# dusk-network/plonk

Hardware: AMD Instinct MI355X
Metric: prove() wall-clock (ms) at 2^20 gates (lower is better)
Workload: dtype u32 limbs (Fr 256-bit / Fp 384-bit Montgomery)

## Files before the change

### include/plonk_hip.h

```cpp
#ifndef PLONK_HIP_H
#define PLONK_HIP_H
#include <stdint.h>

#ifdef __cplusplus
extern "C" {
#endif

typedef struct plonk_ctx plonk_ctx;

enum {
  PLONK_OK = 0,
  PLONK_ERR_ARG = -1,
  PLONK_ERR_HIP = -2,
  PLONK_ERR_DEGREE = -3,
  PLONK_ERR_NO_SRS = -4,
  PLONK_ERR_NO_GPU = -5,
  PLONK_ERR_UNSAT = -6,
  PLONK_ERR_STATE = -7,
  PLONK_ERR_BYTES = -8,
  PLONK_ERR_DATA = -9,
  PLONK_ERR_POINT = -10,
  PLONK_ERR_NOMEM = -11,
  PLONK_ERR_VERIFY = -12
};

int plonk_ctx_create(plonk_ctx** out, const int* devices, int ndev);
void plonk_ctx_destroy(plonk_ctx* ctx);
const char* plonk_last_error(void);

enum { PLONK_TABLE_AUTO = 0, PLONK_TABLE_WINDOW = 16, PLONK_TABLE_HALFPOS = 128, PLONK_TABLE_BITPOS = 256 };
typedef struct plonk_gpu_config {
  uint32_t struct_size;
  uint32_t reserved;
  uint64_t table_budget_bytes;
  int32_t table_mode;
  int32_t msm_bucket_bits;
  int32_t quotient_domain;
  int32_t wire_commit;
  int32_t shard_quotient;
  int32_t shard_grand_product;
  int32_t shard_side_stream;
  int32_t ntt_elements_log2;
  int32_t comm_timeout_ms;
  int32_t side_stream_cus;
} plonk_gpu_config;
int plonk_ctx_create_ex(plonk_ctx** out, int device, const plonk_gpu_config* config );
int plonk_ctx_get_config(plonk_ctx* ctx, plonk_gpu_config* out );
int plonk_ctx_set_config(plonk_ctx* ctx, const plonk_gpu_config* config);

enum { PLONK_PLAN_TAIL_SERIAL = 1, PLONK_PLAN_BUCKET_SUM_LANE = 2, PLONK_PLAN_ACCUMULATE_LDS = 4, PLONK_PLAN_SORT13 = 8 };
typedef struct plonk_msm_plan {
  uint32_t table_rows;
  uint32_t bucket_bits;
  uint32_t digit_width;
  uint32_t slice_entries;
  uint32_t ordered_lanes;
  uint32_t wide_words;
  uint32_t flags;
  uint32_t reserved;
  uint64_t terms;
  char accumulate_kernel[64];
} plonk_msm_plan;
int plonk_ctx_describe_msm(plonk_ctx* ctx, uint64_t m, int count, int bit_sum_tail, uint32_t table_rows, uint64_t table_points,
                           plonk_msm_plan* out);
int plonk_ctx_last_msm(plonk_ctx* ctx, plonk_msm_plan* out);
int plonk_ctx_table_bytes(plonk_ctx* ctx, uint64_t* in_use, uint64_t* budget);

int plonk_ntt(plonk_ctx* ctx, uint64_t* a, uint32_t log_n, int inverse, int coset, uint64_t in_len);
int plonk_ntt_batch(plonk_ctx* ctx, uint64_t* const* a, int count, uint32_t log_n, int inverse,
                    int coset, const uint64_t* in_len);

int plonk_srs_load(plonk_ctx* ctx, const uint8_t* xy96, uint64_t npoints);
int plonk_host_alloc(uint64_t bytes, void** out);
int plonk_host_free(void* p);

int plonk_msm(plonk_ctx* ctx, const uint64_t* scalars, uint64_t m, uint8_t out_xy_inf[97]);
int plonk_msm_batch(plonk_ctx* ctx, const uint64_t* const* scalars, const uint64_t* m, int count,
                    uint8_t* out );

int plonk_ntt_dev(plonk_ctx* ctx, const void* src, void* dst, void* tmp, uint32_t log_n,
                  int inverse, int coset, uint64_t in_len);
int plonk_msm_dev(plonk_ctx* ctx, const void* scalars, uint64_t m, void* out97_dev);
int plonk_srs_load_dev(plonk_ctx* ctx, const void* xy96_dev, uint64_t npoints);
int plonk_srs_generate_dev(plonk_ctx* ctx, const uint64_t tau[4], const uint64_t g_scalar[4],
                           uint64_t npoints, void* out_dev);
int plonk_lagrange_key(plonk_ctx* ctx, uint32_t log_n, uint8_t* out_xy96);

int plonk_dev_alloc(plonk_ctx* ctx, uint64_t bytes, void** out);
int plonk_dev_free(plonk_ctx* ctx, void* p);
int plonk_dev_h2d(plonk_ctx* ctx, void* dst_dev, const void* src_host, uint64_t bytes);
int plonk_dev_d2h(plonk_ctx* ctx, void* dst_host, const void* src_dev, uint64_t bytes);
int plonk_dev_sync(plonk_ctx* ctx);
void* plonk_ctx_stream(plonk_ctx* ctx);
int plonk_ctx_table_rows(plonk_ctx* ctx);

typedef struct plonk_prover plonk_prover;
typedef int (*plonk_allgather_fn)(void* user, const void* send, void* recv, uint64_t bytes_per_rank);
typedef struct {
  uint64_t constraints;
  const uint8_t* label;
  uint64_t label_len;
  const uint64_t* polys[15];
  uint64_t poly_len[15];
  const uint8_t* vk_commitments;
  int shard_rank;
  int shard_world;
  uint64_t srs_total;
  plonk_allgather_fn allgather;
  void* allgather_user;
  const uint8_t* lagrange_xy96;
  uint64_t lagrange_count;
} plonk_prover_desc;
int plonk_prover_create(plonk_ctx* ctx, const plonk_prover_desc* desc, plonk_prover** out);
void plonk_prover_destroy(plonk_prover* p);
int plonk_prover_set_version(plonk_prover* p, int version);
int plonk_prover_vk(plonk_prover* p, uint8_t out[15 * 48]);
typedef struct plonk_prover_info {
  uint64_t size;
  uint32_t quotient_domain;
  uint32_t wire_commit_values;
  uint32_t lagrange_table_rows;
  uint32_t shard_world, shard_rank;
  uint32_t sharded_quotient;
  uint32_t quotient_classes;
  uint32_t wire_group_launches;
  uint64_t lagrange_points;
} plonk_prover_info;
int plonk_prover_describe(plonk_prover* p, plonk_prover_info* out);
uint64_t plonk_prover_size(plonk_prover* p);
int plonk_prover_peek(plonk_prover* p, int which, uint64_t offset, uint64_t count, uint64_t* out);
int plonk_prover_prove(plonk_prover* p, const uint64_t* const wires[4], const uint64_t* pi_idx,
                       const uint64_t* pi_val, uint64_t pi_count, const uint64_t* blinders,
                       uint8_t proof[1008]);
int plonk_prover_prove_dev(plonk_prover* p, const void* wires_dev, const uint64_t* pi_idx,
                           const uint64_t* pi_val, uint64_t pi_count, const uint64_t* blinders,
                           uint8_t proof[1008]);

typedef struct {
  uint64_t constraints;
  const uint8_t* label;
  uint64_t label_len;
  const uint64_t* selectors[11];
  const uint32_t* wires[4];
  uint64_t witnesses;
  int shard_rank;
  int shard_world;
  uint64_t srs_total;
  plonk_allgather_fn allgather;
  void* allgather_user;
  const uint8_t* lagrange_xy96;
  uint64_t lagrange_count;
} plonk_circuit_desc;
int plonk_compile(plonk_ctx* ctx, const plonk_circuit_desc* circuit, plonk_prover** out);
int plonk_prover_prove_witnesses(plonk_prover* p, const uint64_t* witnesses, uint64_t count, const uint64_t* pi_idx,
                                 const uint64_t* pi_val, uint64_t pi_count, const uint64_t* blinders,
                                 uint8_t proof[1008]);

typedef struct plonk_unsat_row {
  uint64_t row;
  uint32_t families;
  uint32_t copy_wires;
} plonk_unsat_row;
typedef struct plonk_unsat_info {
  uint64_t rows_checked;
  uint64_t rows_failing;
  uint64_t family_rows[18];
  uint64_t first_row;
  uint32_t first_family;
  uint32_t reserved;
  double ms;
} plonk_unsat_info;
int plonk_prover_diagnose(plonk_prover* p, const uint64_t* const wires[4], const uint64_t* pi_idx,
                          const uint64_t* pi_val, uint64_t pi_count, plonk_unsat_row* out, uint64_t cap,
                          plonk_unsat_info* info);
int plonk_prover_diagnose_dev(plonk_prover* p, const void* wires_dev, const uint64_t* pi_idx,
                              const uint64_t* pi_val, uint64_t pi_count, plonk_unsat_row* out, uint64_t cap,
                              plonk_unsat_info* info);
int plonk_prover_diagnose_witnesses(plonk_prover* p, const uint64_t* witnesses, uint64_t count, const uint64_t* pi_idx,
                                    const uint64_t* pi_val, uint64_t pi_count, plonk_unsat_row* out, uint64_t cap,
                                    plonk_unsat_info* info);

int plonk_comm_set_library(const char* path);
int plonk_comm_library(char* out, uint64_t cap);
int plonk_comm_measure_loopback(plonk_ctx* ctx, int on);
int plonk_comm_unique_id(uint8_t out[128]);
int plonk_comm_init(plonk_ctx* ctx, const uint8_t unique_id[128], int rank, int world);
int plonk_comm_info(plonk_ctx* ctx, int* rank, int* world);
int plonk_comm_warning(plonk_ctx* ctx, char* out, uint64_t cap);
int plonk_comm_selftest(plonk_ctx* ctx);
int plonk_comm_destroy(plonk_ctx* ctx);

int plonk_prover_to_bytes(plonk_prover* p, uint8_t* out, uint64_t cap, uint64_t* len);
int plonk_verifier_to_bytes(plonk_prover* p, const uint8_t* opening_key, uint64_t opening_key_len,
                            const uint64_t* pi_idx, uint64_t pi_count, uint8_t* out, uint64_t cap, uint64_t* len);
typedef struct plonk_verifier plonk_verifier;
typedef struct {
  uint64_t proofs, msm_terms;
  uint32_t pairing_checks, rejected;
  double ms_decode, ms_scalars, ms_msm, ms_pairing;
} plonk_verify_info;
int plonk_verifier_from_bytes(plonk_ctx* ctx, const uint8_t* blob, uint64_t len, plonk_verifier** out);
void plonk_verifier_destroy(plonk_verifier* v);
int plonk_verifier_set_version(plonk_verifier* v, int version);
int plonk_verify(plonk_verifier* v, const uint8_t* proofs, const uint64_t* pi, uint64_t pi_count, uint64_t count,
                 int32_t* verdicts);
int plonk_verifier_last(plonk_verifier* v, plonk_verify_info* out);
int plonk_verify_mixed(plonk_verifier* const* verifiers, uint32_t nverifiers, const uint32_t* circuit, const uint8_t* proofs,
                       const uint64_t* pi, uint64_t pi_total, uint64_t count, int32_t* verdicts, plonk_verify_info* info);
typedef struct {
  uint64_t size, constraints;
  uint64_t label_off, label_len;
  uint64_t poly_off[15], poly_len[15];
// ... 79 lines not shown
```

### plonk_amd/__init__.py

```python
from __future__ import annotations

import ctypes
import os
import weakref
from typing import Iterable, Sequence

os.environ.setdefault("HSA_ENABLE_IPC_MODE_LEGACY", "0")

_HERE = os.path.dirname(os.path.abspath(__file__))
LIB_PATH = os.environ.get("PLONK_HIP_LIB") or os.path.join(_HERE, "lib", "libplonk_hip.so")

Q = 0x73EDA753299D7D483339D80809A1D80553BDA402FFFE5BFEFFFFFFFF00000001
P = 0x1A0111EA397FE69A4B1BA7B6434BACD764774B84F38512BF6730D2A0F6B0F6241EABFFFEB153FFFFB9FEFFFFFFFFAAAB
_FR_R = (1 << 256) % Q
_FR_RINV = pow(_FR_R, -1, Q)
_FP_R = (1 << 384) % P
_FP_RINV = pow(_FP_R, -1, P)

PLONK_OK = 0
ERRORS = {
    -1: "PLONK_ERR_ARG", -2: "PLONK_ERR_HIP", -3: "PLONK_ERR_DEGREE (PolynomialDegreeTooLarge)",
    -4: "PLONK_ERR_NO_SRS", -5: "PLONK_ERR_NO_GPU", -6: "PLONK_ERR_UNSAT (CircuitUnsatisfied)",
    -7: "PLONK_ERR_STATE", -8: "PLONK_ERR_BYTES (NotEnoughBytes)", -9: "PLONK_ERR_DATA (InvalidData)",
    -10: "PLONK_ERR_POINT (PointMalformed)", -11: "PLONK_ERR_NOMEM (host allocation failed inside the library)",
    -12: "PLONK_ERR_VERIFY (ProofVerificationError)",
}

EXPORTS = [
    "plonk_ctx_create", "plonk_ctx_destroy", "plonk_last_error", "plonk_ntt", "plonk_ntt_batch",
    "plonk_srs_load", "plonk_msm", "plonk_msm_batch", "plonk_ntt_dev", "plonk_msm_dev",
    "plonk_srs_load_dev", "plonk_srs_generate_dev", "plonk_dev_alloc", "plonk_dev_free",
    "plonk_dev_h2d", "plonk_dev_d2h", "plonk_dev_sync", "plonk_ctx_stream", "plonk_ctx_table_rows",
    "plonk_profile_enable", "plonk_profile_read", "plonk_profile_reset",
    "plonk_prover_create", "plonk_prover_destroy", "plonk_prover_vk", "plonk_prover_size",
    "plonk_prover_prove", "plonk_prover_prove_dev", "plonk_prover_peek",
    "plonk_prover_blob_check", "plonk_prover_from_bytes", "plonk_srs_validate",
    "plonk_comm_unique_id", "plonk_comm_init", "plonk_comm_info", "plonk_comm_selftest", "plonk_comm_destroy",
    "plonk_comm_measure_loopback", "plonk_comm_warning", "plonk_prover_set_version", "plonk_comm_set_library", "plonk_comm_library",
    "plonk_ctx_create_ex", "plonk_ctx_get_config", "plonk_ctx_set_config", "plonk_ctx_describe_msm", "plonk_ctx_last_msm",
    "plonk_ctx_table_bytes", "plonk_prover_describe",
    "plonk_host_alloc", "plonk_host_free", "plonk_lagrange_key",
    "plonk_compile", "plonk_prover_prove_witnesses", "plonk_prover_to_bytes", "plonk_verifier_to_bytes",
    "plonk_public_parameters_check", "plonk_srs_load_public_parameters",
    "plonk_verifier_from_bytes", "plonk_verifier_destroy", "plonk_verifier_set_version", "plonk_verify", "plonk_verifier_last",
    "plonk_verify_mixed",
    "plonk_prover_diagnose", "plonk_prover_diagnose_dev", "plonk_prover_diagnose_witnesses",
    "plonk_kzg_open", "plonk_kzg_open_dev", "plonk_kzg_flatten", "plonk_kzg_key_create", "plonk_kzg_key_destroy",
    "plonk_kzg_batch_check", "plonk_srs_check",
    "plonk_composer_create", "plonk_composer_destroy", "plonk_composer_witness", "plonk_composer_gate", "plonk_composer_gadget",
    "plonk_composer_info", "plonk_composer_layout", "plonk_compile_composer",
    "plonk_prover_fill_inputs", "plonk_prover_prove_inputs", "plonk_prover_diagnose_inputs",
]

IDENTITY_FAMILIES = [
    "arithmetic gate",
    "range: quad c - 4d", "range: quad b - 4c", "range: quad a - 4b", "range: quad next d - 4a",
    "logic: left quad", "logic: right quad", "logic: output quad", "logic: product of the input quads", "logic: xor/and relation",
    "fixed-base: scalar bit", "fixed-base: xy of the bit", "fixed-base: x accumulator", "fixed-base: y accumulator",
    "curve addition: x1 y2", "curve addition: x3", "curve addition: y3",
    "copy constraint",
]

POLY_ORDER = ["q_m", "q_l", "q_r", "q_o", "q_f", "q_c", "q_arith", "q_range", "q_logic",
              "q_fixed_group_add", "q_variable_group_add", "s_sigma_1", "s_sigma_2", "s_sigma_3", "s_sigma_4"]


TABLE_AUTO, TABLE_WINDOW, TABLE_HALFPOS, TABLE_BITPOS = 0, 16, 128, 256
PLAN_TAIL_SERIAL, PLAN_BUCKET_SUM_LANE, PLAN_ACCUMULATE_LDS, PLAN_SORT13 = 1, 2, 4, 8


class GpuConfig(ctypes.Structure):
    _fields_ = [("struct_size", ctypes.c_uint32), ("reserved", ctypes.c_uint32), ("table_budget_bytes", ctypes.c_uint64),
                ("table_mode", ctypes.c_int32), ("msm_bucket_bits", ctypes.c_int32), ("quotient_domain", ctypes.c_int32),
                ("wire_commit", ctypes.c_int32), ("shard_quotient", ctypes.c_int32), ("shard_grand_product", ctypes.c_int32),
                ("shard_side_stream", ctypes.c_int32), ("ntt_elements_log2", ctypes.c_int32), ("comm_timeout_ms", ctypes.c_int32),
                ("side_stream_cus", ctypes.c_int32)]

    def __init__(self, **kw):
        super().__init__(**kw)
        self.struct_size = ctypes.sizeof(GpuConfig)

    def as_dict(self) -> dict:
        return {k: getattr(self, k) for k, _ in self._fields_ if k not in ("struct_size", "reserved")}


class _MsmPlan(ctypes.Structure):
    _fields_ = [("table_rows", ctypes.c_uint32), ("bucket_bits", ctypes.c_uint32), ("digit_width", ctypes.c_uint32),
                ("slice_entries", ctypes.c_uint32), ("ordered_lanes", ctypes.c_uint32), ("wide_words", ctypes.c_uint32),
                ("flags", ctypes.c_uint32), ("reserved", ctypes.c_uint32), ("terms", ctypes.c_uint64), ("accumulate_kernel", ctypes.c_char * 64)]

    def as_dict(self) -> dict:
        d = {k: getattr(self, k) for k, _ in self._fields_}
        d["accumulate_kernel"] = d["accumulate_kernel"].decode()
        return d


class _ProverInfo(ctypes.Structure):
    _fields_ = [("size", ctypes.c_uint64), ("quotient_domain", ctypes.c_uint32), ("wire_commit_values", ctypes.c_uint32),
                ("lagrange_table_rows", ctypes.c_uint32), ("shard_world", ctypes.c_uint32), ("shard_rank", ctypes.c_uint32),
                ("sharded_quotient", ctypes.c_uint32), ("quotient_classes", ctypes.c_uint32), ("wire_group_launches", ctypes.c_uint32),
                ("lagrange_points", ctypes.c_uint64)]


class _ProverDesc(ctypes.Structure):
    _fields_ = [("constraints", ctypes.c_uint64), ("label", ctypes.c_char_p), ("label_len", ctypes.c_uint64),
                ("polys", ctypes.c_void_p * 15), ("poly_len", ctypes.c_uint64 * 15),
                ("vk_commitments", ctypes.c_char_p), ("shard_rank", ctypes.c_int), ("shard_world", ctypes.c_int),
                ("srs_total", ctypes.c_uint64), ("allgather", ctypes.c_void_p), ("allgather_user", ctypes.c_void_p),
                ("lagrange_xy96", ctypes.c_char_p), ("lagrange_count", ctypes.c_uint64)]


class _CircuitDesc(ctypes.Structure):
    _fields_ = [("constraints", ctypes.c_uint64), ("label", ctypes.c_char_p), ("label_len", ctypes.c_uint64),
                ("selectors", ctypes.c_void_p * 11), ("wires", ctypes.c_void_p * 4), ("witnesses", ctypes.c_uint64),
                ("shard_rank", ctypes.c_int), ("shard_world", ctypes.c_int),
                ("srs_total", ctypes.c_uint64), ("allgather", ctypes.c_void_p), ("allgather_user", ctypes.c_void_p),
                ("lagrange_xy96", ctypes.c_char_p), ("lagrange_count", ctypes.c_uint64)]


class _UnsatRow(ctypes.Structure):
    _fields_ = [("row", ctypes.c_uint64), ("families", ctypes.c_uint32), ("copy_wires", ctypes.c_uint32)]


class _UnsatInfo(ctypes.Structure):
    _fields_ = [("rows_checked", ctypes.c_uint64), ("rows_failing", ctypes.c_uint64), ("family_rows", ctypes.c_uint64 * 18),
                ("first_row", ctypes.c_uint64), ("first_family", ctypes.c_uint32), ("reserved", ctypes.c_uint32),
                ("ms", ctypes.c_double)]


class Diagnosis:

    def __init__(self, rc: int, rows, info: "_UnsatInfo"):
        self.ok = rc == PLONK_OK
        self.rows = rows
        self.rows_checked, self.rows_failing = info.rows_checked, info.rows_failing
        self.family_rows = list(info.family_rows)
        self.first_row, self.first_family = info.first_row, info.first_family
        self.ms = info.ms

    @property
    def info(self) -> dict:
        return dict(rows_checked=self.rows_checked, rows_failing=self.rows_failing, family_rows=self.family_rows,
                    first_row=self.first_row, first_family=self.first_family)

    def __repr__(self):
        if self.ok:
            return f"Diagnosis(ok, {self.rows_checked} rows)"
        return (f"Diagnosis({self.rows_failing} of {self.rows_checked} rows fail; first: row {self.first_row}, "
                f"{IDENTITY_FAMILIES[self.first_family]})")


class _ComposerSummary(ctypes.Structure):
    _fields_ = [("constraints", ctypes.c_uint64), ("witnesses", ctypes.c_uint64), ("inputs", ctypes.c_uint64),
                ("public_rows", ctypes.c_uint64), ("records", ctypes.c_uint64), ("levels", ctypes.c_uint64),
                ("widest_level", ctypes.c_uint64)]


class _BlobInfo(ctypes.Structure):
    _fields_ = [("size", ctypes.c_uint64), ("constraints", ctypes.c_uint64), ("label_off", ctypes.c_uint64),
                ("label_len", ctypes.c_uint64), ("poly_off", ctypes.c_uint64 * 15), ("poly_len", ctypes.c_uint64 * 15),
                ("srs_off", ctypes.c_uint64), ("srs_points", ctypes.c_uint64), ("vk_off", ctypes.c_uint64)]


class _VerifyInfo(ctypes.Structure):
    _fields_ = [("proofs", ctypes.c_uint64), ("msm_terms", ctypes.c_uint64), ("pairing_checks", ctypes.c_uint32),
                ("rejected", ctypes.c_uint32), ("ms_decode", ctypes.c_double), ("ms_scalars", ctypes.c_double),
                ("ms_msm", ctypes.c_double), ("ms_pairing", ctypes.c_double)]


class KzgProof(ctypes.Structure):
    _fields_ = [("commitment", ctypes.c_uint8 * 48), ("evaluation", ctypes.c_uint64 * 4), ("witness", ctypes.c_uint8 * 48)]

    @classmethod
    def make(cls, commitment: bytes, evaluation: int, witness: bytes) -> "KzgProof":
        p = cls()
        ctypes.memmove(p.commitment, bytes(commitment), 48)
        ctypes.memmove(p.evaluation, fr_to_bytes_mont([evaluation]), 32)
        ctypes.memmove(p.witness, bytes(witness), 48)
        return p

    @property
    def value(self) -> int:
        return fr_from_bytes_mont(bytes(self.evaluation))[0]


class _PublicParametersInfo(ctypes.Structure):
    _fields_ = [("opening_key_off", ctypes.c_uint64), ("points_off", ctypes.c_uint64), ("point_stride", ctypes.c_uint64),
                ("points_total", ctypes.c_uint64), ("points_kept", ctypes.c_uint64)]


PP_RAW_UNCHECKED, PP_RAW, PP_COMPRESSED = 0, 1, 2


ALLGATHER_FN = ctypes.CFUNCTYPE(ctypes.c_int, ctypes.c_void_p, ctypes.c_void_p, ctypes.c_void_p, ctypes.c_uint64)


def shard_range(total: int, rank: int, world: int) -> tuple[int, int]:
    per = (total + world - 1) // world
    lo = min(per * rank, total)
    return lo, min(lo + per, total)


class CircuitUnsatisfied(Exception):
    """Mirrors Error::CircuitUnsatisfied (reference quotient_poly.rs:132)."""


class PlonkError(RuntimeError):
    def __init__(self, code: int, detail: str = ""):
        self.code = code
        super().__init__(f"{ERRORS.get(code, code)} {detail}".strip())


class NotEnoughBytes(PlonkError):
    """Mirrors Error::NotEnoughBytes (reference prover.rs:274,310; widget.rs:484; key.rs:265,281)."""


class InvalidData(PlonkError):
    """Mirrors dusk_bytes::Error::InvalidData as the reference's decoders raise it."""


class PointMalformed(PlonkError):
    """Mirrors Error::PointMalformed (reference key.rs:292)."""


_DECODE_ERRORS = {-8: NotEnoughBytes, -9: InvalidData, -10: PointMalformed}


class ProofVerificationError(PlonkError):
    """Mirrors Error::ProofVerificationError (reference proof.rs:502-512): plonk_verify's PLONK_ERR_VERIFY."""


class PolynomialDegreeTooLarge(PlonkError):
    """Mirrors Error::PolynomialDegreeTooLarge (reference key.rs:362-370)."""


_lib = None


def load_library() -> ctypes.CDLL:
    global _lib
    if _lib is not None:
        return _lib
# ... 1071 lines not shown
```

### plonk_amd/csrc/capi.hip

```cpp
#include <chrono>
#include <cstdio>
#include <cstring>
#include <sched.h>
#include <thread>

#include "plonk_internal.hpp"
#include "hostg1.hpp"

namespace plonk {

static thread_local char g_last_error[512] = "";

void set_last_error(const char* what, const char* detail, const char* file, int line) {
  snprintf(g_last_error, sizeof g_last_error, "%s:%d: %s -> %s", file, line, what ? what : "?", detail ? detail : "?");
}

int srs_generate_device(Ctx* c, const Fr& tau, const Fr& g_scalar, uint64_t n, G1Affine* out_dev);

int ctx_refuse_poisoned(const char* api_fn) {
  set_last_error(api_fn, "context unusable: a collective timed out and its stream never drained (comm_sync); destroy the context", __FILE__, __LINE__);
  return PLONK_ERR_STATE;
}

bool ctx_abandon(Ctx* c) {
// ... 220 lines not shown
  if (c.wire_commit != 0 && c.wire_commit != 1) return bad("plonk_gpu_config.wire_commit");
  if (c.ntt_elements_log2 != 0 && c.ntt_elements_log2 != 2 && c.ntt_elements_log2 != 3) return bad("plonk_gpu_config.ntt_elements_log2");
  for (int v : {c.shard_quotient, c.shard_grand_product, c.shard_side_stream}) if (v < -1 || v > 1) return bad("plonk_gpu_config.shard_*: -1, 0 or 1");
  if (c.comm_timeout_ms < 0 || c.side_stream_cus < -1 || c.side_stream_cus > 200) return bad("plonk_gpu_config.comm_timeout_ms / side_stream_cus");
  return PLONK_OK;
}

static int side_stream_partition(Ctx* c) {
  const int k = c->cfg.side_cus;
  if (k <= 0) return PLONK_OK;
  hipDeviceProp_t prop;
  HIP_TRY(hipGetDeviceProperties(&prop, c->device));
  const int ncu = prop.multiProcessorCount;
  if (k >= ncu) return (set_last_error("plonk_gpu_config.side_stream_cus", "must be smaller than the device's compute-unit count", __FILE__, __LINE__), PLONK_ERR_ARG);
  const int words = (ncu + 31) / 32;
  std::vector<uint32_t> side(words, 0u);
  for (int i = 0; i < ncu; ++i)
    if ((int64_t)i * k / ncu != (int64_t)(i + 1) * k / ncu) side[i / 32] |= 1u << (i % 32);
  hipStream_t ss = nullptr;
  if (hipExtStreamCreateWithCUMask(&ss, (uint32_t)words, side.data()) != hipSuccess) return (set_last_error("hipExtStreamCreateWithCUMask", "side stream", __FILE__, __LINE__), PLONK_ERR_HIP);
  (void)hipStreamDestroy(c->side_stream);
  c->side_stream = ss;
  return PLONK_OK;
}

}

extern "C" {

const char* plonk_last_error(void) { return g_last_error; }

static int create_context(plonk_ctx** out, int dev, const plonk_gpu_config* config, const char* api_fn) {
  if (!out) return PLONK_ERR_ARG;
  { const int rc = config_check(config, api_fn); if (rc) return rc; }
  int count = 0;
  if (hipGetDeviceCount(&count) != hipSuccess || count == 0) {
    set_last_error("hipGetDeviceCount", "no HIP device visible", __FILE__, __LINE__);
    return PLONK_ERR_NO_GPU;
  }
  if (dev < 0 || dev >= count) return PLONK_ERR_ARG;
  HIP_TRY(hipSetDevice(dev));
  auto* ctx = new plonk_ctx();
  ctx->c.device = dev;
  config_resolve(config, dev, &ctx->c.cfg);
  int prio_least = 0, prio_greatest = 0;
  (void)hipDeviceGetStreamPriorityRange(&prio_least, &prio_greatest);
  hipError_t e = hipStreamCreateWithPriority(&ctx->c.stream, hipStreamNonBlocking, prio_greatest);
  if (e == hipSuccess) e = hipStreamCreateWithPriority(&ctx->c.side_stream, hipStreamNonBlocking, prio_least);
  ctx->c.main_stream = ctx->c.stream;
  if (e != hipSuccess) {
    set_last_error("hipStreamCreate", hipGetErrorString(e), __FILE__, __LINE__);
    delete ctx;
    return PLONK_ERR_HIP;
  }
  { const int rc = side_stream_partition(&ctx->c); if (rc) { (void)hipStreamDestroy(ctx->c.stream); (void)hipStreamDestroy(ctx->c.side_stream); delete ctx; return rc; } }
  *out = ctx;
  return PLONK_OK;
}

int plonk_ctx_create(plonk_ctx** out, const int* devices, int ndev) {
  const char* const api_fn = __func__;
  return plonk::api_guard(api_fn, [&]() -> int {
  if (!out || ndev > 1 || ndev < 0) return PLONK_ERR_ARG;
  return create_context(out, (devices && ndev == 1) ? devices[0] : 0, nullptr, api_fn);
  });
}

int plonk_ctx_create_ex(plonk_ctx** out, int device, const plonk_gpu_config* config) {
  const char* const api_fn = __func__;
  return plonk::api_guard(api_fn, [&]() -> int { return create_context(out, device, config, api_fn); });
}

int plonk_ctx_get_config(plonk_ctx* ctx, plonk_gpu_config* out) {
  const char* const api_fn = __func__;
  return plonk::api_guard(api_fn, [&]() -> int {
  if (!ctx || !out || out->struct_size < 8 || out->struct_size > 4096) return (set_last_error("invalid argument", "plonk_ctx_get_config: set struct_size = sizeof(plonk_gpu_config)", __FILE__, __LINE__), PLONK_ERR_ARG);
  std::lock_guard<std::mutex> lk(ctx->c.mu);
  const Config& g = ctx->c.cfg;
  plonk_gpu_config full{};
  full.struct_size = (uint32_t)sizeof(plonk_gpu_config);
  full.table_budget_bytes = g.table_budget;
  full.table_mode = g.table_mode;
  full.msm_bucket_bits = g.bucket_bits;
  full.quotient_domain = g.quotient_domain;
  full.wire_commit = g.wire_commit_coeff;
  full.shard_quotient = g.shard_quotient;
  full.shard_grand_product = g.shard_z;
  full.shard_side_stream = g.shard_side;
  full.ntt_elements_log2 = g.ntt_elog;
  full.comm_timeout_ms = g.comm_timeout_ms;
  full.side_stream_cus = g.side_cus;
  const uint32_t want = out->struct_size < sizeof(full) ? out->struct_size : (uint32_t)sizeof(full);
  memcpy(out, &full, want);
  out->struct_size = want;
  return PLONK_OK;
  });
}

int plonk_ctx_set_config(plonk_ctx* ctx, const plonk_gpu_config* config) {
  const char* const api_fn = __func__;
  return plonk::api_guard(api_fn, [&]() -> int {
  if (!ctx) return PLONK_ERR_ARG;
  { const int rc = config_check(config, api_fn); if (rc) return rc; }
  std::lock_guard<std::mutex> lk(ctx->c.mu);
  Config next;
  config_resolve(config, ctx->c.device, &next);
  if (next.side_cus != ctx->c.cfg.side_cus)
    return (set_last_error("plonk_ctx_set_config", "side_stream_cus can only be chosen at plonk_ctx_create_ex", __FILE__, __LINE__), PLONK_ERR_STATE);
  ctx->c.cfg = next;
  return PLONK_OK;
  });
}

int plonk_ctx_table_bytes(plonk_ctx* ctx, uint64_t* in_use, uint64_t* budget) {
  const char* const api_fn = __func__;
  return plonk::api_guard(api_fn, [&]() -> int {
  if (!ctx) return PLONK_ERR_ARG;
  std::lock_guard<std::mutex> lk(ctx->c.mu);
  if (in_use) *in_use = ctx->c.table_bytes;
  if (budget) *budget = ctx->c.cfg.table_budget;
  return PLONK_OK;
  });
}

static void plan_out(const plonk_msm_plan_internal& p, plonk_msm_plan* out) {
  memset(out, 0, sizeof(*out));
  out->table_rows = p.table_rows; out->bucket_bits = p.bucket_bits; out->digit_width = p.digit_width;
  out->slice_entries = p.slice_entries; out->ordered_lanes = p.ordered_lanes; out->wide_words = p.wide_words; out->flags = p.flags; out->terms = p.terms;
  snprintf(out->accumulate_kernel, sizeof(out->accumulate_kernel), "%s", p.kernel);
}

int plonk_ctx_describe_msm(plonk_ctx* ctx, uint64_t m, int count, int bit_sum_tail, uint32_t table_rows, uint64_t table_points, plonk_msm_plan* out) {
  const char* const api_fn = __func__;
  return plonk::api_guard(api_fn, [&]() -> int {
  if (!ctx || !out || count < 1 || count > MSM_MAX_BATCH) return PLONK_ERR_ARG;
  std::lock_guard<std::mutex> lk(ctx->c.mu);
  Ctx& c = ctx->c;
  if (table_rows == 0) { table_rows = c.srs_rows; table_points = c.srs_n; if (!c.srs_table) return PLONK_ERR_NO_SRS; }
  if (table_rows != MSM_ROWS_WINDOW && table_rows != MSM_ROWS_HALFPOS && table_rows != MSM_ROWS_BITPOS) return PLONK_ERR_ARG;
  plonk_msm_plan_internal p;
  msm_plan(&c, table_rows, table_points, m, count, bit_sum_tail != 0, &p);
  plan_out(p, out);
  return PLONK_OK;
  });
}

int plonk_ctx_last_msm(plonk_ctx* ctx, plonk_msm_plan* out) {
  const char* const api_fn = __func__;
  return plonk::api_guard(api_fn, [&]() -> int {
  if (!ctx || !out) return PLONK_ERR_ARG;
  std::lock_guard<std::mutex> lk(ctx->c.mu);
  if (!ctx->c.last_plan.table_rows) return (set_last_error("plonk_ctx_last_msm", "no MSM has run on this context", __FILE__, __LINE__), PLONK_ERR_STATE);
  plan_out(ctx->c.last_plan, out);
  return PLONK_OK;
  });
}

void plonk_ctx_destroy(plonk_ctx* ctx) {
  if (!ctx) return;
  (void)plonk_comm_destroy(ctx);
  Ctx& c = ctx->c;
  finish_pool_release(&c);
  (void)hipSetDevice(c.device);
  if (ctx_abandon(&c)) {
    prof_forget(&c);
    delete ctx;
    return;
  }
  (void)hipStreamSynchronize(c.stream);
  verify_ws_release(&c);
  kzg_ws_release(&c);
  for (auto& kv : c.ntt_tables) {
    NttTables* t = kv.second;
    (void)hipFree(t->tw_lo); (void)hipFree(t->tw_hi); (void)hipFree(t->tw_lo_scaled);
    (void)hipFree(t->w512); (void)hipFree(t->g_lo); (void)hipFree(t->g_hi);
    (void)hipFree(t->tw_lo29); (void)hipFree(t->tw_hi29); (void)hipFree(t->tw_lo_scaled29);
    (void)hipFree(t->w512_29); (void)hipFree(t->g_lo29); (void)hipFree(t->g_hi29);
    (void)hipFree(t->tw_a29); (void)hipFree(t->tw_b29);
    delete t;
  }
  (void)hipFree(c.ntt_buf); (void)hipFree(c.ntt_buf2); (void)hipFree(c.ntt_buf3); (void)hipFree(c.ntt_tmp);
  if (c.down_stream) (void)hipStreamDestroy(c.down_stream);
  if (c.copy_stream) (void)hipStreamDestroy(c.copy_stream); (void)hipFree(c.srs_table); (void)hipFree(c.table_scratch);
  MsmWork& w = c.msm;
  (void)hipFree(w.tmp_words); (void)hipFree(w.entries); (void)hipFree(w.coarse_cnt); (void)hipFree(w.coarse_off); (void)hipFree(w.coarse_cur); (void)hipFree(w.big_off); (void)hipFree(w.big_cnt); (void)hipFree(w.nheavy); (void)hipFree(w.heavy_list); (void)hipFree(w.seg_sum);
  (void)hipFree(w.offsets); (void)hipFree(w.slice_off); (void)hipFree(w.full_off); (void)hipFree(w.part_list); (void)hipFree(w.partial); (void)hipFree(w.buckets);
  (void)hipFree(w.multi_list); (void)hipFree(w.layout);
  (void)hipFree(w.chunk); (void)hipFree(w.result); (void)hipFree(w.scalars_stage);
  if (w.result_host) (void)hipHostFree(w.result_host);
  prof_release(&c);
  (void)hipStreamDestroy(c.main_stream);
  if (c.side_stream) (void)hipStreamDestroy(c.side_stream);
  delete ctx;
}

int plonk_ctx_table_rows(plonk_ctx* ctx) { return ctx ? (int)ctx->c.srs_rows : 0; }
void* plonk_ctx_stream(plonk_ctx* ctx) { return ctx ? (void*)ctx->c.main_stream : nullptr; }

int plonk_dev_alloc(plonk_ctx* ctx, uint64_t bytes, void** out) {
  const char* const api_fn = __func__;
  return plonk::api_guard(api_fn, [&]() -> int {
  if (!ctx || !out) return PLONK_ERR_ARG;
  HIP_TRY(hipSetDevice(ctx->c.device));
  HIP_TRY(hipMalloc(out, bytes ? bytes : 1));
  return PLONK_OK;
  });
}
int plonk_dev_free(plonk_ctx* ctx, void* p) {
  const char* const api_fn = __func__;
  return plonk::api_guard(api_fn, [&]() -> int {
  if (!ctx) return PLONK_ERR_ARG;
  CTX_ENTER(ctx->c, api_fn);
  HIP_TRY(hipSetDevice(ctx->c.device));
  HIP_TRY(hipStreamSynchronize(ctx->c.main_stream));
  HIP_TRY(hipFree(p));
  return PLONK_OK;
  });
}
int plonk_dev_h2d(plonk_ctx* ctx, void* dst, const void* src, uint64_t bytes) {
  const char* const api_fn = __func__;
  return plonk::api_guard(api_fn, [&]() -> int {
  if (!ctx || (!dst && bytes) || (!src && bytes)) return PLONK_ERR_ARG;
  CTX_ENTER(ctx->c, api_fn);
  HIP_TRY(hipSetDevice(ctx->c.device));
  HIP_TRY(hipMemcpyAsync(dst, src, bytes, hipMemcpyHostToDevice, ctx->c.main_stream));
  HIP_TRY(hipStreamSynchronize(ctx->c.main_stream));
  return PLONK_OK;
  });
}
int plonk_dev_d2h(plonk_ctx* ctx, void* dst, const void* src, uint64_t bytes) {
  const char* const api_fn = __func__;
  return plonk::api_guard(api_fn, [&]() -> int {
  if (!ctx || (!dst && bytes) || (!src && bytes)) return PLONK_ERR_ARG;
  CTX_ENTER(ctx->c, api_fn);
  HIP_TRY(hipSetDevice(ctx->c.device));
  HIP_TRY(hipMemcpyAsync(dst, src, bytes, hipMemcpyDeviceToHost, ctx->c.main_stream));
  HIP_TRY(hipStreamSynchronize(ctx->c.main_stream));
  return PLONK_OK;
  });
}
int plonk_dev_sync(plonk_ctx* ctx) {
  const char* const api_fn = __func__;
  return plonk::api_guard(api_fn, [&]() -> int {
  if (!ctx) return PLONK_ERR_ARG;
  CTX_ENTER(ctx->c, api_fn);
  HIP_TRY(hipSetDevice(ctx->c.device));
  HIP_TRY(hipStreamSynchronize(ctx->c.main_stream));
  return PLONK_OK;
  });
}

int plonk_ntt_dev(plonk_ctx* ctx, const void* src, void* dst, void* tmp, uint32_t log_n, int inverse,
                  int coset, uint64_t in_len) {
  const char* const api_fn = __func__;
  return plonk::api_guard(api_fn, [&]() -> int {
  if (!ctx || !src || !dst || log_n >= 28) return PLONK_ERR_ARG;
  if (log_n > 10 && !tmp) return PLONK_ERR_ARG;
  CTX_ENTER(ctx->c, api_fn);
  HIP_TRY(hipSetDevice(ctx->c.device));
  prof_begin(&ctx->c, 0);
  int rc = ntt_device(&ctx->c, (const Fr*)src, (Fr*)dst, (Fr*)tmp, log_n, inverse != 0, coset != 0, in_len);
  prof_end(&ctx->c, 0);
  return rc;
  });
}

int plonk_ntt(plonk_ctx* ctx, uint64_t* a, uint32_t log_n, int inverse, int coset, uint64_t in_len) {
  const char* const api_fn = __func__;
  return plonk::api_guard(api_fn, [&]() -> int {
  if (!ctx || !a || log_n >= 28) return PLONK_ERR_ARG;
  Ctx& c = ctx->c;
  CTX_ENTER(c, api_fn);
  HIP_TRY(hipSetDevice(c.device));
  const uint64_t n = 1ull << log_n;
  if (in_len > n) in_len = n;
  int rc = ensure_ntt_staging(&c, n);
  if (rc) return rc;
  HIP_TRY(hipMemcpyAsync(c.ntt_buf, a, sizeof(Fr) * in_len, hipMemcpyHostToDevice, c.stream));
  rc = ntt_device(&c, c.ntt_buf, c.ntt_buf, c.ntt_tmp, log_n, inverse != 0, coset != 0, in_len);
  if (rc) return rc;
  HIP_TRY(hipMemcpyAsync(a, c.ntt_buf, sizeof(Fr) * n, hipMemcpyDeviceToHost, c.stream));
  HIP_TRY(hipStreamSynchronize(c.stream));
  return PLONK_OK;
  });
}

int plonk_ntt_batch(plonk_ctx* ctx, uint64_t* const* a, int count, uint32_t log_n, int inverse, int coset,
                    const uint64_t* in_len) {
  const char* const api_fn = __func__;
  return plonk::api_guard(api_fn, [&]() -> int {
  if (!ctx || !a || count < 0 || log_n >= 28) return PLONK_ERR_ARG;
  for (int i = 0; i < count; ++i) if (!a[i]) return PLONK_ERR_ARG;
  if (count == 0) return PLONK_OK;
  Ctx& c = ctx->c;
  CTX_ENTER(c, api_fn);
  HIP_TRY(hipSetDevice(c.device));
  const uint64_t n = 1ull << log_n;
  int rc = ensure_ntt_staging(&c, n);
  if (rc) return rc;
  if (!c.copy_stream) HIP_TRY(hipStreamCreateWithFlags(&c.copy_stream, hipStreamNonBlocking));
  if (!c.down_stream) HIP_TRY(hipStreamCreateWithFlags(&c.down_stream, hipStreamNonBlocking));
  Fr* buf[3] = {c.ntt_buf, c.ntt_buf2, c.ntt_buf3};
  hipEvent_t up[3] = {nullptr, nullptr, nullptr}, done[3] = {nullptr, nullptr, nullptr}, freed[3] = {nullptr, nullptr, nullptr};
  hipError_t e = hipSuccess;
  for (int k = 0; k < 3 && e == hipSuccess; ++k) {
    e = hipEventCreateWithFlags(&up[k], hipEventDisableTiming);
    if (e == hipSuccess) e = hipEventCreateWithFlags(&done[k], hipEventDisableTiming);
    if (e == hipSuccess) e = hipEventCreateWithFlags(&freed[k], hipEventDisableTiming);
  }
  for (int k = 0; k < count && e == hipSuccess && rc == PLONK_OK; ++k) {
    const int b = k % 3;
    uint64_t len = in_len ? in_len[k] : n;
    if (len > n) len = n;
    if (k >= 3) e = hipStreamWaitEvent(c.copy_stream, freed[b], 0);
    if (e == hipSuccess) e = hipMemcpyAsync(buf[b], a[k], sizeof(Fr) * len, hipMemcpyHostToDevice, c.copy_stream);
    if (e == hipSuccess) e = hipEventRecord(up[b], c.copy_stream);
    if (e == hipSuccess) e = hipStreamWaitEvent(c.stream, up[b], 0);
    if (e == hipSuccess) rc = ntt_device(&c, buf[b], buf[b], c.ntt_tmp, log_n, inverse != 0, coset != 0, len);
    if (e == hipSuccess && rc == PLONK_OK) e = hipEventRecord(done[b], c.stream);
    if (e == hipSuccess && rc == PLONK_OK) e = hipStreamWaitEvent(c.down_stream, done[b], 0);
    if (e == hipSuccess && rc == PLONK_OK) e = hipMemcpyAsync(a[k], buf[b], sizeof(Fr) * n, hipMemcpyDeviceToHost, c.down_stream);
    if (e == hipSuccess && rc == PLONK_OK) e = hipEventRecord(freed[b], c.down_stream);
  }
  const hipError_t e1 = hipStreamSynchronize(c.copy_stream), e2 = hipStreamSynchronize(c.stream), e3 = hipStreamSynchronize(c.down_stream);
  if (e == hipSuccess) e = e1 != hipSuccess ? e1 : (e2 != hipSuccess ? e2 : e3);
  for (int k = 0; k < 3; ++k) {
    if (up[k]) (void)hipEventDestroy(up[k]);
    if (done[k]) (void)hipEventDestroy(done[k]);
    if (freed[k]) (void)hipEventDestroy(freed[k]);
  }
  if (e != hipSuccess) { set_last_error("plonk_ntt_batch", hipGetErrorString(e), __FILE__, __LINE__); if (rc == PLONK_OK) rc = PLONK_ERR_HIP; }
  return rc;
  });
}

int plonk_srs_load_dev(plonk_ctx* ctx, const void* xy96_dev, uint64_t npoints) {
  const char* const api_fn = __func__;
  return plonk::api_guard(api_fn, [&]() -> int {
// ... 238 lines not shown
```

### plonk_amd/csrc/msm.hip

```cpp
#include <cstdlib>

#include "plonk_internal.hpp"
#include "curve28.cuh"
#include "fr29.cuh"

namespace plonk {


static constexpr uint32_t MSM_KSL = 32;
static constexpr uint32_t MSM_CHUNK = 16;

__device__ __forceinline__ Fr ld_fr_g(const Fr* p) {
  const uint4* q = reinterpret_cast<const uint4*>(p);
  uint4 a = q[0], b = q[1];
  Fr r;
  r.l[0] = a.x; r.l[1] = a.y; r.l[2] = a.z; r.l[3] = a.w;
  r.l[4] = b.x; r.l[5] = b.y; r.l[6] = b.z; r.l[7] = b.w;
  return r;
}
__device__ __forceinline__ Fp ld_fp(const Fp* p) {
  const uint4* q = reinterpret_cast<const uint4*>(p);
  uint4 a = q[0], b = q[1], c = q[2];
  Fp r;
  r.l[0] = a.x; r.l[1] = a.y; r.l[2] = a.z; r.l[3] = a.w;
// ... 1135 lines not shown
  if (MSM_NB_BITS > 15 && !bit_sums) return (plonk::set_last_error("msm", "the 2^19-bucket variant only emits bit sums", __FILE__, __LINE__), PLONK_ERR_ARG);
  {
    const uint64_t avg_slices = (MSM_W * mmax) / bt.ksl / MSM_NB;
    bt.heavy_thresh = (uint32_t)(2 * avg_slices > 16 ? 2 * avg_slices : 16);
  }
  const bool fine = c->cfg.prof_fine;
  const int fbase = bt.group_count >= 3 ? 16 : 24;
#define FINE_BEGIN(ph) do { if (fine) prof_begin(c, fbase + (ph)); } while (0)
#define FINE_END(ph) do { if (fine) prof_end(c, fbase + (ph)); } while (0)
  const bool tail_quad = !c->cfg.tail_serial;
  if (phase & 1) {
  bt.ordered = (msm_acc_ordered(c, bt.ksl) && !c->cfg.acc_lds) ? 1u : 0u;
  prof_begin(c, 2);
  FINE_BEGIN(0);
  rc = msm_group_sort(c, bt, mmax);
  FINE_END(0);
  prof_end(c, 2);
  if (rc) return rc;
  const uint64_t max_slices = (MSM_W * mmax) / bt.ksl + MSM_NB + 1;
  prof_begin(c, 1);
  FINE_BEGIN(1);
  const bool acc_lds = c->cfg.acc_lds;
  const bool acc_ordered = msm_acc_ordered(c, bt.ksl);
  if (acc_ordered && !acc_lds) {
    rc = msm_order_slices(c, bt);
    if (rc) return rc;
    const uint32_t acc_wg = c->cfg.acc_wg == 64 ? 64u : 128u;
    hipLaunchKernelGGL(msm_accumulate_ordered_kernel, dim3((uint32_t)((max_slices + acc_wg - 1) / acc_wg), count), dim3(acc_wg), 0, st,
                       (const G1AffineR*)table, bt, w.entries, w.offsets, w.slice_off, w.full_off, w.part_list, (G1RSlot*)w.partial, (G1RSlot*)w.buckets);
  } else if (acc_lds)
    hipLaunchKernelGGL(msm_accumulate_lds_kernel, dim3((uint32_t)((max_slices + 127) / 128), count), dim3(128), 0, st,
                       (const G1AffineR*)table, bt, w.entries, w.offsets, w.slice_off, (G1RSlot*)w.partial);
  else
    hipLaunchKernelGGL(msm_accumulate_kernel, dim3((uint32_t)((max_slices + 127) / 128), count), dim3(128), 0, st,
                       (const G1AffineR*)table, bt, w.entries, w.offsets, w.slice_off, (G1RSlot*)w.partial);
  FINE_END(1);
  prof_end(c, 1);
  if (c->acc_done) HIP_TRY(hipEventRecord(c->acc_done, st));
  prof_begin(c, 2);
  FINE_BEGIN(2);
  {
    const uint64_t avg_slices = (MSM_W * mmax) / bt.ksl / MSM_NB;
    const uint32_t heavy_thresh = bt.heavy_thresh;
    const bool tail_quad_ = !c->cfg.tail_serial;
    const uint32_t fused = (tail_quad_ || MSM_NB_BITS > 15) ? HEAVY_FUSED_WGS : 0u;
    const bool list_mode = MSM_NB_BITS > 15 && acc_ordered && !acc_lds;
    const bool bsum_lane = c->cfg.bsum_lane;
    const bool dense_quad = !list_mode && tail_quad_ && !bsum_lane && avg_slices <= 8;
#define BSUM(G) hipLaunchKernelGGL(msm_bucket_sum_kernel<G>, dim3((list_mode ? 1024u : (dense_quad ? MSM_NB * 4 / 128 : MSM_NB * G / 128)) + fused, count), dim3(128), 0, st, bt, \
                                   (const G1RSlot*)w.partial, w.slice_off, (G1RSlot*)w.buckets, heavy_thresh, w.nheavy, (const HeavyItem*)w.heavy_list, \
                                   (G1RSlot*)w.seg_sum, w.cap_segs, fused, (acc_ordered && !acc_lds) ? 1u : 0u, \
                                   list_mode ? (const uint32_t*)w.multi_list : (const uint32_t*)nullptr, dense_quad ? 1u : 0u)
    if (dense_quad) BSUM(1);
    else if (avg_slices <= 4) BSUM(1);
    else if (avg_slices <= 16) BSUM(2);
    else if (avg_slices <= 32) BSUM(4);
    else BSUM(8);
#undef BSUM
  }
  FINE_END(2);
  FINE_BEGIN(3);
  if (tail_quad || MSM_NB_BITS > 15) {
    hipLaunchKernelGGL(msm_heavy_bucket_quad_kernel, dim3(256, count), dim3(256), 0, st, w.nheavy, (const HeavyItem*)w.heavy_list,
                       (const G1RSlot*)w.seg_sum, w.cap_segs, (G1RSlot*)w.buckets, HEAVY_FUSED_WGS, bt.kb0);
  } else {
    hipLaunchKernelGGL(msm_heavy_seg_kernel, dim3(4 * HEAVY_WGS, count), dim3(64), 0, st, bt, (const G1RSlot*)w.partial, w.slice_off,
                       w.nheavy, (const HeavyItem*)w.heavy_list, (G1RSlot*)w.seg_sum, w.cap_segs);
    hipLaunchKernelGGL(msm_heavy_bucket_kernel, dim3(256, count), dim3(256), 0, st, w.nheavy, (const HeavyItem*)w.heavy_list,
                       (const G1RSlot*)w.seg_sum, w.cap_segs, (G1RSlot*)w.buckets, bt.kb0);
  }
  FINE_END(3);
  if (!(phase & 2)) { prof_end(c, 2); HIP_TRY(hipGetLastError()); return PLONK_OK; }
  } else {
    prof_begin(c, 2);
  }
  bt.kb0 = 0;
  bt.count = bt.group_count;
  const int count_g = bt.group_count;
  c->msm.last_rowbits = 8 + (MSM_NB_BITS - 15);
#if PLONK_MSM_NB_BITS > 15
  {
    G1RSlot* rc1 = (G1RSlot*)w.chunk;
    G1RSlot* rc2 = rc1 + (size_t)TP_RC1 * MSM_MAX_BATCH;
    const bool rc_lane_tree = c->cfg.rc_lane_tree;
#define TPK(LPS) do { if (rc_lane_tree) hipLaunchKernelGGL((msm_rowcol_tp_kernel<LPS, false>), dim3(TP_ROWS * LPS / 128 + TP_PARTS * LPS, count_g), dim3(128), 0, st, (const G1RSlot*)w.buckets, rc1); \
                      else hipLaunchKernelGGL((msm_rowcol_tp_kernel<LPS, true>), dim3(TP_ROWS * LPS / 128 + TP_PARTS * LPS, count_g), dim3(128), 0, st, (const G1RSlot*)w.buckets, rc1); } while (0)
    const int lps_env = c->cfg.lps;
    int lps = count_g >= 2 ? 8 : 16;
    if (MSM_NB_BITS == 17) lps = count_g >= 3 ? 16 : 32;
    if (lps_env == 4 || lps_env == 8 || lps_env == 16 || lps_env == 32) lps = lps_env;
    else if (lps_env == 1) lps = count_g >= 3 ? 8 : (count_g == 2 ? 16 : 32);
    FINE_BEGIN(4);
    if (lps == 4) TPK(4); else if (lps == 8) TPK(8); else if (lps == 16) TPK(16); else TPK(32);
#undef TPK
    hipLaunchKernelGGL(msm_fold_quad_kernel, dim3(256 + TP_NP + 128, count_g), dim3(64), 0, st, (const G1RSlot*)rc1, rc2);
    FINE_END(4);
    FINE_BEGIN(5);
    hipLaunchKernelGGL(msm_bits_quad_kernel, dim3(17 + TP_E, count_g), dim3(256), 0, st, bt, (const G1RSlot*)rc2, (uint32_t)TP_RC2, (uint32_t)TP_E);
    FINE_END(5);
    prof_end(c, 2);
    HIP_TRY(hipGetLastError());
    return PLONK_OK;
  }
#else
  if (bit_sums && tail_quad) {
    FINE_BEGIN(4);
    const int rcwv_env = c->cfg.rcwv;
    int wv = count_g >= 3 ? 1 : (count_g == 2 ? 2 : 4);
    if (rcwv_env >= 111) wv = count_g >= 3 ? rcwv_env % 10 : (count_g == 2 ? (rcwv_env / 10) % 10 : rcwv_env / 100);
    if (wv == 1) hipLaunchKernelGGL(msm_rowcol_quad_kernel<1>, dim3(RCQ_SUMS, count_g), dim3(64), 0, st, (const G1RSlot*)w.buckets, (G1RSlot*)w.chunk);
    else if (wv == 2) hipLaunchKernelGGL(msm_rowcol_quad_kernel<2>, dim3(RCQ_SUMS, count_g), dim3(128), 0, st, (const G1RSlot*)w.buckets, (G1RSlot*)w.chunk);
    else hipLaunchKernelGGL(msm_rowcol_quad_kernel<4>, dim3(RCQ_SUMS, count_g), dim3(256), 0, st, (const G1RSlot*)w.buckets, (G1RSlot*)w.chunk);
    FINE_END(4);
    FINE_BEGIN(5);
    hipLaunchKernelGGL(msm_bits_quad_kernel, dim3(17, count_g), dim3(256), 0, st, bt, (const G1RSlot*)w.chunk, (uint32_t)RCQ_SUMS, 0u);
    FINE_END(5);
    prof_end(c, 2);
    HIP_TRY(hipGetLastError());
    return PLONK_OK;
  }
  hipLaunchKernelGGL(msm_rowcol_kernel, dim3(RC_WG, count_g), dim3(256), 0, st, (const G1RSlot*)w.buckets,
                     (G1RSlot*)w.chunk);
  if (bit_sums) {
    hipLaunchKernelGGL(msm_bits_kernel, dim3(17, count_g), dim3(128), 0, st, bt, (const G1RSlot*)w.chunk);
  } else {
    constexpr size_t smem = sizeof(G1R) * (RC_ROWS + RC_COLS);
    smem_opt_in(c, (const void*)msm_final_kernel, smem);
    hipLaunchKernelGGL(msm_final_kernel, dim3(count_g), dim3(384), smem, st, bt, (const G1RSlot*)w.chunk);
  }
  prof_end(c, 2);
  HIP_TRY(hipGetLastError());
  return PLONK_OK;
#endif
#undef FINE_BEGIN
#undef FINE_END
}


}

#if PLONK_MSM_NB_BITS == 15
static uint64_t msm_slice_cap(const Ctx* c, uint64_t cap) {
  if (c->cfg.ksl >= 4) return (uint64_t)MSM_W * cap / c->cfg.ksl + MSM_NB_MAX + 1;
  const uint64_t nb15 = 1ull << 15;
  const uint64_t small = (uint64_t)MSM_W * cap / 4 < (uint64_t)MSM_W * nb15 ? (uint64_t)MSM_W * cap / 4 : (uint64_t)MSM_W * nb15;
  const uint64_t large = (uint64_t)MSM_W * cap / MSM_KSL;
  return (small > large ? small : large) + MSM_NB_MAX + 1;
}

int msm_sort_reserve_fixed(Ctx* c) {
  MsmWork& w = c->msm;
  constexpr int KB = MSM_MAX_BATCH;
  constexpr uint32_t COARSE = 2048;
  HIP_TRY(hipMalloc((void**)&w.coarse_cnt, sizeof(uint32_t) * COARSE * KB));
  HIP_TRY(hipMalloc((void**)&w.coarse_off, sizeof(uint32_t) * (COARSE + 1) * KB));
  HIP_TRY(hipMalloc((void**)&w.coarse_cur, sizeof(uint32_t) * COARSE * KB));
  HIP_TRY(hipMalloc((void**)&w.big_off, sizeof(uint32_t) * (COARSE + 1) * KB));
  HIP_TRY(hipMalloc((void**)&w.big_cnt, sizeof(uint32_t) * 2 * MSM_NB_MAX * KB));
  HIP_TRY(hipMalloc((void**)&w.full_off, sizeof(uint32_t) * (MSM_NB_MAX + 1) * KB));
  HIP_TRY(hipMalloc((void**)&w.part_list, sizeof(uint32_t) * (MSM_NB_MAX + 1) * KB));
  HIP_TRY(hipMalloc((void**)&w.multi_list, sizeof(uint32_t) * MSM_NB_MAX * KB));
  HIP_TRY(hipMalloc((void**)&w.layout, sizeof(uint32_t) * (2 * (MSM_NB_MAX / 1024) + (MSM_NB_MAX / 1024 + 1) * 132) * KB));
  return PLONK_OK;
}

int msm_reserve(Ctx* c, uint64_t m) {
  MsmWork& w = c->msm;
  constexpr int KB = MSM_MAX_BATCH;
  if (!w.fixed_ok) {
    for (void** q : {(void**)&w.offsets, (void**)&w.slice_off, (void**)&w.nheavy, &w.heavy_list, (void**)&w.coarse_cnt, (void**)&w.coarse_off,
                     (void**)&w.coarse_cur, (void**)&w.big_off, (void**)&w.big_cnt, (void**)&w.full_off, (void**)&w.part_list, (void**)&w.layout, (void**)&w.multi_list, &w.buckets, &w.chunk,
                     (void**)&w.result}) {
      if (*q) { (void)hipFree(*q); *q = nullptr; }
    }
    if (w.result_host) { (void)hipHostFree(w.result_host); w.result_host = nullptr; }
    HIP_TRY(hipMalloc((void**)&w.offsets, sizeof(uint32_t) * (MSM_NB_MAX + 1) * KB));
    HIP_TRY(hipMalloc((void**)&w.slice_off, sizeof(uint32_t) * (MSM_NB_MAX + 1) * KB));
    HIP_TRY(hipMalloc((void**)&w.nheavy, sizeof(uint32_t) * 4 * KB));
    HIP_TRY(hipMalloc((void**)&w.heavy_list, sizeof(HeavyItem) * MSM_NB_MAX * KB));
    { const int rc_s = msm_sort_reserve_fixed(c); if (rc_s) return rc_s; }
    HIP_TRY(hipMalloc((void**)&w.buckets, sizeof(G1RSlot) * MSM_NB_MAX * KB));
    HIP_TRY(hipMalloc((void**)&w.chunk, sizeof(G1RSlot) * (2 * (MSM_NB_MAX / 128) + 1024) * KB));
    HIP_TRY(hipMalloc((void**)&w.result, sizeof(G1) * MSM_BIT_SUMS * KB));
    HIP_TRY(hipHostMalloc((void**)&w.result_host, sizeof(G1) * MSM_BIT_SUMS * KB, hipHostMallocDefault));
    w.fixed_ok = true;
  }
  if (m > w.cap_m || msm_slice_cap(c, w.cap_m) > w.cap_slices) {
    const uint64_t cap = m > w.cap_m ? m : w.cap_m;
    HIP_TRY(hipStreamSynchronize(c->stream));
    w.cap_m = 0;
    for (void** q : {(void**)&w.tmp_words, (void**)&w.entries, (void**)&w.partial, &w.seg_sum}) {
      if (*q) { HIP_TRY(hipFree(*q)); *q = nullptr; }
    }
    HIP_TRY(hipMalloc((void**)&w.tmp_words, sizeof(uint64_t) * MSM_W * cap * KB));
    HIP_TRY(hipMalloc((void**)&w.entries, sizeof(uint32_t) * MSM_W * cap * KB));
    w.cap_slices = msm_slice_cap(c, cap);
    HIP_TRY(hipMalloc((void**)&w.partial, sizeof(G1RSlot) * w.cap_slices * KB));
    w.cap_segs = w.cap_slices / 128 + MSM_NB_MAX + 1;
    HIP_TRY(hipMalloc((void**)&w.seg_sum, sizeof(G1RSlot) * w.cap_segs * KB));
    w.cap_m = cap;
  }
  return PLONK_OK;
}

void msm_plan(const Ctx* c, uint32_t table_rows, uint64_t table_n, uint64_t mmax, int count, bool bit_sums, plonk_msm_plan_internal* out) {
  (void)count;
  const int buckets_env = c->cfg.bucket_bits;
  const bool can_large = (table_rows == MSM_ROWS_BITPOS || table_rows == MSM_ROWS_HALFPOS) && bit_sums && !c->cfg.tail_serial && !c->cfg.acc_lds;
  int nb_bits = 15;
  if (can_large) {
    if (buckets_env == 17 || buckets_env == 19) nb_bits = buckets_env;
    else if (buckets_env > 15) nb_bits = 19;
    else if (buckets_env != 15) nb_bits = mmax > (1ull << 18) + 64 ? 19 : 15;
  }
#ifndef PLONK_MSM_WITH_MEDIUM
  if (nb_bits == 17) nb_bits = 19;
#endif
  plonk_msm_plan_internal p;
  p.table_rows = table_rows;
  p.bucket_bits = (uint32_t)nb_bits;
  p.digit_width = table_rows == MSM_ROWS_WINDOW ? 16u : (table_rows == MSM_ROWS_BITPOS ? (uint32_t)nb_bits + 2u : (uint32_t)nb_bits + 1u);
  p.terms = mmax;
  bool ordered;
  if (nb_bits == 19) { p.slice_entries = nbl::msm_ksl(c, mmax); ordered = nbl::msm_acc_ordered(c, p.slice_entries); p.wide_words = nbl::msm_needs_wide_words(table_rows, table_n); }
#ifdef PLONK_MSM_WITH_MEDIUM
  else if (nb_bits == 17) { p.slice_entries = nbm::msm_ksl(c, mmax); ordered = nbm::msm_acc_ordered(c, p.slice_entries); p.wide_words = nbm::msm_needs_wide_words(table_rows, table_n); }
#endif
  else { p.slice_entries = nb15::msm_ksl(c, mmax); ordered = nb15::msm_acc_ordered(c, p.slice_entries); p.wide_words = nb15::msm_needs_wide_words(table_rows, table_n); }
  p.ordered_lanes = ordered && !c->cfg.acc_lds;
  static const char* const names[3][3] = {
      {"nb15::msm_accumulate_kernel", "nb15::msm_accumulate_ordered_kernel", "nb15::msm_accumulate_lds_kernel"},
      {"nbm::msm_accumulate_kernel", "nbm::msm_accumulate_ordered_kernel", "nbm::msm_accumulate_lds_kernel"},
      {"nbl::msm_accumulate_kernel", "nbl::msm_accumulate_ordered_kernel", "nbl::msm_accumulate_lds_kernel"}};
  const uint64_t avg_slices = (MSM_W * mmax) / (p.slice_entries ? p.slice_entries : 1) / (1ull << nb_bits);
  p.flags = ((nb_bits > 15 && c->cfg.sort13 == 1) ? PLONK_PLAN_SORT13 : 0u) | (c->cfg.tail_serial ? PLONK_PLAN_TAIL_SERIAL : 0u) | (c->cfg.acc_lds ? PLONK_PLAN_ACCUMULATE_LDS : 0u) |
            ((c->cfg.bsum_lane || c->cfg.tail_serial || avg_slices > 8 || (nb_bits > 15 && p.ordered_lanes)) ? PLONK_PLAN_BUCKET_SUM_LANE : 0u);
  p.kernel = names[nb_bits == 19 ? 2 : (nb_bits == 17 ? 1 : 0)][c->cfg.acc_lds ? 2 : (p.ordered_lanes ? 1 : 0)];
  *out = p;
}

int msm_batch_device(Ctx* c, const Fr* const* scalars_dev, const uint64_t* m, int count, G1* const* out_dev, bool bit_sums,
                     const void* table, uint64_t table_n, const Fr* const* tail_dev, const uint64_t* split, uint32_t table_rows,
                     int phase, int kb0, int kcount) {
  if (count <= 0) return PLONK_OK;
  if (count > MSM_MAX_BATCH) return (plonk::set_last_error("invalid argument", __func__, __FILE__, __LINE__), PLONK_ERR_ARG);
  if (kcount < 0) kcount = count - kb0;
  if (phase < 1 || phase > 3 || kb0 < 0 || kcount < 1 || kb0 + kcount > count || (phase == 3 && (kb0 != 0 || kcount != count)))
    return (plonk::set_last_error("invalid argument", "msm_batch_device: phase / column range", __FILE__, __LINE__), PLONK_ERR_ARG);
  if (!table) { table = c->srs_table; table_n = c->srs_n; table_rows = c->srs_rows; }
  if (table && table_rows != MSM_ROWS_WINDOW && table_rows != MSM_ROWS_BITPOS && table_rows != MSM_ROWS_HALFPOS) return (plonk::set_last_error("invalid argument", "msm: table rows", __FILE__, __LINE__), PLONK_ERR_ARG);
  uint64_t mmax = 0;
  for (int k = 0; k < count; ++k) {
    if (m[k] > table_n) return PLONK_ERR_DEGREE;
    if (m[k] > mmax) mmax = m[k];
  }
  hipStream_t st = c->stream;
  if (mmax == 0) {
    if (!(phase & 2)) return PLONK_OK;
    c->msm.last_rowbits = 8;
    for (int k = 0; k < count; ++k)
      for (int j = 0; j < (bit_sums ? MSM_BIT_SUMS : 1); ++j) hipLaunchKernelGGL(msm_identity_kernel, dim3(1), dim3(64), 0, st, out_dev[k] + j);
    HIP_TRY(hipGetLastError());
    if (c->acc_done) HIP_TRY(hipEventRecord(c->acc_done, st));
    return PLONK_OK;
  }
  if (!table) return PLONK_ERR_NO_SRS;
  int rc = msm_reserve(c, mmax);
  if (rc) return rc;
  MsmWork& w = c->msm;
  MsmBatch bt{};
  bt.count = (phase & 1) ? kcount : count;
  bt.kb0 = (phase & 1) ? kb0 : 0;
  bt.group_count = count;
  bt.cap_m = w.cap_m;
  bt.cap_slices = w.cap_slices;
  bt.table = table;
  bt.table_n = table_n;
  bt.rows = table_rows;
  for (int k = 0; k < count; ++k) {
    bt.scalars[k] = scalars_dev[k]; bt.m[k] = m[k]; bt.out[k] = out_dev[k];
    bt.tail[k] = tail_dev ? tail_dev[k] : nullptr;
    bt.split[k] = (tail_dev && split) ? split[k] : ~0ull;
  }
  plonk_msm_plan_internal plan;
  msm_plan(c, table_rows, table_n, mmax, count, bit_sums, &plan);
  c->last_plan = plan;
  const int nb_bits = (int)plan.bucket_bits;
  if (nb_bits == 19) return nbl::msm_batch_device_v(c, bt, mmax, bit_sums, phase);
#ifdef PLONK_MSM_WITH_MEDIUM
  if (nb_bits == 17) return nbm::msm_batch_device_v(c, bt, mmax, bit_sums, phase);
#else
  if (nb_bits == 17) return nbl::msm_batch_device_v(c, bt, mmax, bit_sums, phase);
#endif
  return nb15::msm_batch_device_v(c, bt, mmax, bit_sums, phase);
}

int msm_device(Ctx* c, const Fr* scalars_dev, uint64_t m, G1* out_dev) {
  return msm_batch_device(c, &scalars_dev, &m, 1, &out_dev, false);
}

int xyzz_to_affine97_device(Ctx* c, const G1* in_dev, uint8_t* out97_dev) {
  hipLaunchKernelGGL(xyzz_to_affine97_kernel, dim3(1), dim3(64), 0, c->stream, in_dev, out97_dev);
  HIP_TRY(hipGetLastError());
  return PLONK_OK;
}
#endif

}
```

### plonk_amd/csrc/msm_sort.hip

```cpp
#include "plonk_internal.hpp"
#include "fr29.cuh"

namespace plonk {
namespace PLONK_MSM_NS {

static constexpr uint32_t FINE_BITS = MSM_NB_BITS - 11;
static constexpr uint32_t COARSE = MSM_NB >> FINE_BITS;
#ifndef PLONK_SORT_TILE
#define PLONK_SORT_TILE 2048
#endif
static constexpr uint32_t TILE = PLONK_SORT_TILE;
static constexpr uint32_t SORT_T = 1024;
static constexpr uint32_t PER_T = TILE / SORT_T;
#ifndef PLONK_HIST_PER
#define PLONK_HIST_PER 2
#endif
static constexpr uint32_t HIST_PER = PLONK_HIST_PER;
static constexpr uint32_t HIST_TILE = SORT_T * HIST_PER;
static_assert(COARSE == 2 * SORT_T, "scan / reservation loops assume two coarse bins per thread");
static constexpr uint32_t IDX_BITS = 31 - FINE_BITS;
static constexpr uint32_t IDX_MASK = (1u << IDX_BITS) - 1;
static_assert(IDX_BITS + 1 + FINE_BITS == 32, "narrow intermediate word layout");
template <class WordT> struct SortWord;
template <> struct SortWord<uint32_t> {
  __device__ static __forceinline__ uint32_t make(uint32_t fine, uint32_t sign, uint64_t idx) { return (fine << (IDX_BITS + 1)) | (sign << IDX_BITS) | (uint32_t)idx; }
  __device__ static __forceinline__ uint32_t fine(uint32_t w) { return w >> (IDX_BITS + 1); }
  __device__ static __forceinline__ uint32_t entry(uint32_t w) { return (w & IDX_MASK) | (((w >> IDX_BITS) & 1u) << 31); }
};
template <> struct SortWord<uint64_t> {
  __device__ static __forceinline__ uint64_t make(uint32_t fine, uint32_t sign, uint64_t idx) { return ((uint64_t)fine << 32) | ((uint64_t)sign << 31) | idx; }
  __device__ static __forceinline__ uint32_t fine(uint64_t w) { return (uint32_t)(w >> 32); }
  __device__ static __forceinline__ uint32_t entry(uint64_t w) { return (uint32_t)w; }
};
template <class WordT> struct TmpPlanes;
template <> struct TmpPlanes<uint32_t> {
  uint32_t* lo;
  __device__ __forceinline__ TmpPlanes(void* all, int kb, uint64_t words) : lo((uint32_t*)all + (uint64_t)kb * words) {}
  __device__ __forceinline__ uint32_t ld(uint32_t j) const { return lo[j]; }
  __device__ __forceinline__ uint32_t ld_fine(uint32_t j) const { return SortWord<uint32_t>::fine(lo[j]); }
  __device__ __forceinline__ void st(uint32_t j, uint32_t w) const { lo[j] = w; }
};
template <> struct TmpPlanes<uint64_t> {
  uint32_t* lo;
  uint8_t* hi;
  __device__ __forceinline__ TmpPlanes(void* all, int kb, uint64_t words)
      : lo((uint32_t*)all + (uint64_t)kb * words), hi((uint8_t*)((uint32_t*)all + (uint64_t)MSM_MAX_BATCH * words) + (uint64_t)kb * words) {}
  __device__ __forceinline__ uint64_t ld(uint32_t j) const { return ((uint64_t)hi[j] << 32) | lo[j]; }
  __device__ __forceinline__ uint32_t ld_fine(uint32_t j) const { return hi[j]; }
  __device__ __forceinline__ void st(uint32_t j, uint64_t w) const { lo[j] = (uint32_t)w; hi[j] = (uint8_t)(w >> 32); }
};
static_assert(TILE <= 2048, "tile-local word: 11 bits of scalar index");

__device__ __forceinline__ Fr ld_scalar(const Fr* p);
__device__ __forceinline__ Fr ld_scalar_at(const MsmBatch& bt, int kb, uint64_t i) {
  return i < bt.split[kb] ? ld_scalar(bt.scalars[kb] + i) : ld_scalar(bt.tail[kb] + (i - bt.split[kb]));
}
__device__ __forceinline__ Fr ld_scalar(const Fr* p) {
  const uint4* q = reinterpret_cast<const uint4*>(p);
  const uint4 a = q[0], b = q[1];
  Fr r;
  r.l[0] = a.x; r.l[1] = a.y; r.l[2] = a.z; r.l[3] = a.w;
  r.l[4] = b.x; r.l[5] = b.y; r.l[6] = b.z; r.l[7] = b.w;
  return r;
}

__device__ __forceinline__ Fr scalar_canonical(const Fr& mont) {
  Fr29 c32 = Fr29::zero();
  c32.l[0] = 32;
  return Fr29::mul(Fr29::from_fr(mont), c32).to_fr();
}

static constexpr uint32_t MSM_EVEN_WIDTH = (MSM_NB_BITS + 1) & ~1u;
template <int MODE>
__global__ void __launch_bounds__(SORT_T) msm_hist_kernel(MsmBatch bt, uint32_t* __restrict__ coarse_cnt_all) {
  constexpr bool BITPOS = MODE != 0;
  __shared__ uint32_t hist[COARSE];
  __shared__ uint32_t park[BITPOS ? 9 * SORT_T : 1];
  const int kb = (int)blockIdx.y + bt.kb0;
  const uint64_t m = bt.m[kb];
  const uint64_t base = (uint64_t)blockIdx.x * HIST_TILE;
  if (base >= m) return;
  const uint32_t t = threadIdx.x;
  hist[t] = 0;
  hist[t + SORT_T] = 0;
  __syncthreads();
  Fr raw[HIST_PER];
#pragma unroll
  for (uint32_t k = 0; k < HIST_PER; ++k) {
    const uint64_t i = base + t + (uint64_t)k * SORT_T;
    if (i < m) raw[k] = ld_scalar_at(bt, kb, i);
  }
#pragma unroll
  for (uint32_t k = 0; k < HIST_PER; ++k) {
    const uint64_t i = base + t + (uint64_t)k * SORT_T;
    if (i < m) {
      const Fr s = scalar_canonical(raw[k]);
      auto count = [&](int, uint32_t, uint32_t bucket, uint32_t) { atomicAdd(&hist[bucket >> FINE_BITS], 1u); };
      if (BITPOS) {
#pragma unroll
        for (int j = 0; j < 8; ++j) park[j * SORT_T + t] = s.l[j];
        park[8 * SORT_T + t] = 0;
        if (MODE == 2) for_each_digit_even<MSM_EVEN_WIDTH>(StridedLimbs{park + t, SORT_T}, count);
        else for_each_digit_naf<MSM_NAF_WIDTH>(StridedLimbs{park + t, SORT_T}, count);
      } else if constexpr (MSM_NB_BITS == 15) {
        for_each_digit_window(s, count);
      }
    }
  }
  __syncthreads();
  uint32_t* __restrict__ cnt = coarse_cnt_all + (uint64_t)kb * COARSE;
  const uint32_t a = hist[t], b = hist[t + SORT_T];
  if (a) atomicAdd(&cnt[t], a);
  if (b) atomicAdd(&cnt[t + SORT_T], b);
}

__device__ __forceinline__ uint32_t block_exclusive_scan(uint32_t v, uint32_t* sh , uint32_t* total) {
  const uint32_t t = threadIdx.x;
  sh[t] = v;
  __syncthreads();
  for (uint32_t d = 1; d < SORT_T; d <<= 1) {
    const uint32_t x = t >= d ? sh[t - d] : 0;
    __syncthreads();
    sh[t] += x;
    __syncthreads();
  }
  const uint32_t incl = sh[t];
  *total = sh[SORT_T - 1];
  __syncthreads();
  return incl - v;
}

__device__ __forceinline__ void fine_exclusive_scan(const uint32_t* cnt, uint32_t* ex, uint32_t* sc, uint32_t* total) {
  constexpr uint32_t NF = 1u << FINE_BITS;
  const uint32_t t = threadIdx.x;
  const uint32_t v = t < NF ? cnt[t] : 0u;
  if (t < NF) sc[t] = v;
  __syncthreads();
  for (uint32_t d = 1; d < NF; d <<= 1) {
    const uint32_t x = (t < NF && t >= d) ? sc[t - d] : 0u;
    __syncthreads();
    if (t < NF) sc[t] += x;
    __syncthreads();
  }
  if (t < NF) ex[t] = sc[t] - v;
  *total = sc[NF - 1];
  __syncthreads();
}

static constexpr uint32_t BIG_LIMIT = 1u << 16;
static constexpr uint32_t BIG_CHUNK = 1u << 14;
__device__ __forceinline__ uint32_t big_chunks(uint32_t cnt) { return cnt > BIG_LIMIT ? (cnt + BIG_CHUNK - 1) / BIG_CHUNK : 0u; }

__global__ void __launch_bounds__(SORT_T) msm_coarse_scan_kernel(const uint32_t* __restrict__ coarse_cnt_all,
                                                                 uint32_t* __restrict__ coarse_off_all,
                                                                 uint32_t* __restrict__ coarse_cur_all,
                                                                 uint32_t* __restrict__ big_off_all, int kb0) {
  __shared__ uint32_t sh[SORT_T];
  const uint32_t* __restrict__ cnt = coarse_cnt_all + (uint64_t)(blockIdx.x + (uint32_t)kb0) * COARSE;
  uint32_t* __restrict__ off = coarse_off_all + (uint64_t)(blockIdx.x + (uint32_t)kb0) * (COARSE + 1);
  uint32_t* __restrict__ cur = coarse_cur_all + (uint64_t)(blockIdx.x + (uint32_t)kb0) * COARSE;
  uint32_t* __restrict__ big = big_off_all + (uint64_t)(blockIdx.x + (uint32_t)kb0) * (COARSE + 1);
  const uint32_t t = threadIdx.x;
  const uint32_t c0 = cnt[2 * t], c1 = cnt[2 * t + 1];
  uint32_t total;
  const uint32_t ex = block_exclusive_scan(c0 + c1, sh, &total);
  off[2 * t] = ex;
  off[2 * t + 1] = ex + c0;
  cur[2 * t] = 0;
  cur[2 * t + 1] = 0;
  if (t == SORT_T - 1) off[COARSE] = total;
  const uint32_t b0 = big_chunks(c0), b1 = big_chunks(c1);
  uint32_t btotal;
  const uint32_t bex = block_exclusive_scan(b0 + b1, sh, &btotal);
  big[2 * t] = bex;
  big[2 * t + 1] = bex + b0;
  if (t == SORT_T - 1) big[COARSE] = btotal;
}

static constexpr size_t PARTITION_LDS = ((size_t)TILE * MSM_W + 3 * COARSE) * sizeof(uint32_t);

template <int MODE, class WordT>
__global__ void __launch_bounds__(SORT_T) msm_partition_kernel(MsmBatch bt, uint64_t srs_n,
                                                               const uint32_t* __restrict__ coarse_off_all,
                                                               uint32_t* __restrict__ coarse_cur_all,
                                                               void* __restrict__ tmp_all) {
  constexpr bool BITPOS = MODE != 0;
  extern __shared__ __attribute__((aligned(16))) uint32_t lds[];
  uint32_t* stage = lds;
  uint32_t* hist = lds + TILE * MSM_W;
  uint32_t* loff = hist + COARSE;
  uint32_t* gbase = loff + COARSE;
  __shared__ uint32_t sh[SORT_T];
  const int kb = (int)blockIdx.y + bt.kb0;
  const uint64_t m = bt.m[kb];
  const uint64_t base = (uint64_t)blockIdx.x * TILE;
  if (base >= m) return;
  const uint32_t t = threadIdx.x;
  hist[t] = 0;
  hist[t + SORT_T] = 0;
  __syncthreads();
  uint32_t word[PER_T][MSM_W], where[PER_T][MSM_W];
#pragma unroll
  for (uint32_t k = 0; k < PER_T; ++k) {
#pragma unroll
    for (int w = 0; w < MSM_W; ++w) where[k][w] = 0xffffffffu;
    const uint64_t i = base + t + (uint64_t)k * SORT_T;
    if (i < m) {
      const Fr s = scalar_canonical(ld_scalar_at(bt, kb, i));
      auto put = [&](int w, uint32_t row, uint32_t bucket, uint32_t sign) {
        const uint32_t bin = bucket >> FINE_BITS;
        const uint32_t rank = atomicAdd(&hist[bin], 1u);
        where[k][w] = (bin << 16) | rank;
        word[k][w] = ((bucket & ((1u << FINE_BITS) - 1)) << 20) | (sign << 19) | (row << 11) | (t + k * SORT_T);
      };
      if (BITPOS) {
        uint32_t* park = stage + k * (9 * SORT_T);
#pragma unroll
        for (int j = 0; j < 8; ++j) park[j * SORT_T + t] = s.l[j];
        park[8 * SORT_T + t] = 0;
        if (MODE == 2) for_each_digit_even<MSM_EVEN_WIDTH>(StridedLimbs{park + t, SORT_T}, put);
        else for_each_digit_naf<MSM_NAF_WIDTH>(StridedLimbs{park + t, SORT_T}, put);
      } else if constexpr (MSM_NB_BITS == 15) {
        for_each_digit_window(s, put);
      }
    }
  }
  __syncthreads();
  {
    const uint32_t c0 = hist[2 * t], c1 = hist[2 * t + 1];
    uint32_t total;
    const uint32_t ex = block_exclusive_scan(c0 + c1, sh, &total);
    loff[2 * t] = ex;
    loff[2 * t + 1] = ex + c0;
    const uint32_t* __restrict__ coff = coarse_off_all + (uint64_t)kb * (COARSE + 1);
    uint32_t* __restrict__ cur = coarse_cur_all + (uint64_t)kb * COARSE;
    gbase[2 * t] = c0 ? coff[2 * t] + atomicAdd(&cur[2 * t], c0) : 0;
    gbase[2 * t + 1] = c1 ? coff[2 * t + 1] + atomicAdd(&cur[2 * t + 1], c1) : 0;
  }
  __syncthreads();
  const TmpPlanes<WordT> tmp(tmp_all, kb, (uint64_t)MSM_W * bt.cap_m);
#pragma unroll
  for (uint32_t k = 0; k < PER_T; ++k)
#pragma unroll
    for (int w = 0; w < MSM_W; ++w)
      if (where[k][w] != 0xffffffffu) stage[loff[where[k][w] >> 16] + (where[k][w] & 0xffffu)] = word[k][w];
  __syncthreads();
  const uint32_t sub = t & 15;
  for (uint32_t bin = t >> 4; bin < COARSE; bin += SORT_T / 16) {
    const uint32_t cnt = hist[bin], lo = loff[bin], gb = gbase[bin];
    for (uint32_t j = sub; j < cnt; j += 16) {
      const uint32_t lw = stage[lo + j];
      tmp.st(gb + j, SortWord<WordT>::make(lw >> 20, (lw >> 19) & 1u, (uint64_t)((lw >> 11) & 0xffu) * srs_n + base + (lw & 0x7ffu)));
    }
  }
}

#if PLONK_MSM_NB_BITS >= 19
static constexpr uint32_t P2_TILE = 1024, P2_T = 512, P2_W = 13, P2_PER = P2_TILE / P2_T, P2_BPT = COARSE / P2_T;
static constexpr size_t PARTITION2_LDS = ((size_t)P2_TILE * P2_W + 3 * COARSE) * sizeof(uint32_t);
static_assert(P2_PER * 9 * P2_T <= P2_TILE * P2_W, "the parked scalars fit the staging area");
static_assert((MSM_NAF_WIDTH) * P2_W >= 256 && (MSM_EVEN_WIDTH) * P2_W >= 256, "13 digit slots cover a scalar");

__device__ __forceinline__ uint32_t block_exclusive_scan_p2(uint32_t v, uint32_t* sh , uint32_t* total) {
  const uint32_t t = threadIdx.x;
  sh[t] = v;
  __syncthreads();
  for (uint32_t d = 1; d < P2_T; d <<= 1) {
    const uint32_t x = t >= d ? sh[t - d] : 0;
    __syncthreads();
    sh[t] += x;
    __syncthreads();
  }
  const uint32_t incl = sh[t];
  *total = sh[P2_T - 1];
  __syncthreads();
  return incl - v;
}

template <int MODE, class WordT>
__global__ void __launch_bounds__(P2_T, 4) msm_partition2_kernel(MsmBatch bt, uint64_t srs_n,
                                                                  const uint32_t* __restrict__ coarse_off_all,
                                                                  uint32_t* __restrict__ coarse_cur_all,
                                                                  void* __restrict__ tmp_all) {
  static_assert(MODE != 0, "bit-position / half-density recodings only");
  extern __shared__ __attribute__((aligned(16))) uint32_t lds[];
  uint32_t* stage = lds;
  uint32_t* hist = lds + P2_TILE * P2_W;
  uint32_t* loff = hist + COARSE;
  uint32_t* gbase = loff + COARSE;
  __shared__ uint32_t sh[P2_T];
  const int kb = (int)blockIdx.y + bt.kb0;
  const uint64_t m = bt.m[kb];
  const uint64_t base = (uint64_t)blockIdx.x * P2_TILE;
  if (base >= m) return;
  const uint32_t t = threadIdx.x;
#pragma unroll
  for (uint32_t j = 0; j < P2_BPT; ++j) hist[t + j * P2_T] = 0;
  __syncthreads();
  uint32_t word[P2_PER][P2_W], where[P2_PER][P2_W];
#pragma unroll
  for (uint32_t k = 0; k < P2_PER; ++k) {
#pragma unroll
    for (uint32_t w = 0; w < P2_W; ++w) where[k][w] = 0xffffffffu;
    const uint64_t i = base + t + (uint64_t)k * P2_T;
    if (i < m) {
      const Fr s = scalar_canonical(ld_scalar_at(bt, kb, i));
      auto put = [&](int w, uint32_t row, uint32_t bucket, uint32_t sign) {
        if (w < (int)P2_W) {
          const uint32_t bin = bucket >> FINE_BITS;
          const uint32_t rank = atomicAdd(&hist[bin], 1u);
          where[k][w] = (bin << 16) | rank;
          word[k][w] = ((bucket & ((1u << FINE_BITS) - 1)) << 20) | (sign << 19) | (row << 11) | (t + k * P2_T);
        }
      };
      uint32_t* park = stage + k * (9 * P2_T);
#pragma unroll
      for (int j = 0; j < 8; ++j) park[j * P2_T + t] = s.l[j];
      park[8 * P2_T + t] = 0;
      if (MODE == 2) for_each_digit_even<MSM_EVEN_WIDTH>(StridedLimbs{park + t, P2_T}, put);
      else for_each_digit_naf<MSM_NAF_WIDTH>(StridedLimbs{park + t, P2_T}, put);
    }
  }
  __syncthreads();
  {
    uint32_t cnt[P2_BPT], sum = 0;
#pragma unroll
    for (uint32_t j = 0; j < P2_BPT; ++j) { cnt[j] = hist[P2_BPT * t + j]; sum += cnt[j]; }
    uint32_t total;
    uint32_t run = block_exclusive_scan_p2(sum, sh, &total);
    const uint32_t* __restrict__ coff = coarse_off_all + (uint64_t)kb * (COARSE + 1);
    uint32_t* __restrict__ cur = coarse_cur_all + (uint64_t)kb * COARSE;
#pragma unroll
    for (uint32_t j = 0; j < P2_BPT; ++j) {
      const uint32_t bin = P2_BPT * t + j;
      loff[bin] = run;
      run += cnt[j];
      gbase[bin] = cnt[j] ? coff[bin] + atomicAdd(&cur[bin], cnt[j]) : 0;
    }
  }
  __syncthreads();
  const TmpPlanes<WordT> tmp(tmp_all, kb, (uint64_t)MSM_W * bt.cap_m);
#pragma unroll
  for (uint32_t k = 0; k < P2_PER; ++k)
#pragma unroll
    for (uint32_t w = 0; w < P2_W; ++w)
      if (where[k][w] != 0xffffffffu) stage[loff[where[k][w] >> 16] + (where[k][w] & 0xffffu)] = word[k][w];
  __syncthreads();
  const uint32_t sub = t & 7;
  for (uint32_t bin = t >> 3; bin < COARSE; bin += P2_T / 8) {
    const uint32_t cnt = hist[bin], lo = loff[bin], gb = gbase[bin];
    for (uint32_t j = sub; j < cnt; j += 8) {
      const uint32_t lw = stage[lo + j];
      tmp.st(gb + j, SortWord<WordT>::make(lw >> 20, (lw >> 19) & 1u, (uint64_t)((lw >> 11) & 0xffu) * srs_n + base + (lw & 0x7ffu)));
    }
  }
}
#endif

#ifndef PLONK_FINE_T
#define PLONK_FINE_T 512
#endif
#ifndef PLONK_FINE_CACHE
#define PLONK_FINE_CACHE 20
#endif
static constexpr uint32_t FINE_T = PLONK_FINE_T;
static constexpr uint32_t FINE_CACHE = PLONK_FINE_CACHE;
template <class WordT>
__global__ void __launch_bounds__(FINE_T) msm_fine_kernel(MsmBatch bt, const uint32_t* __restrict__ coarse_off_all,
                                                          void* __restrict__ tmp_all,
                                                          uint32_t* __restrict__ entries_all,
                                                          uint32_t* __restrict__ offsets_all) {
  __shared__ uint32_t cnt[1u << FINE_BITS], start[1u << FINE_BITS], cur[1u << FINE_BITS], scan_tmp[1u << FINE_BITS];
  const int kb = (int)blockIdx.y + bt.kb0;
  const uint32_t bin = blockIdx.x, t = threadIdx.x;
  const uint32_t* __restrict__ coff = coarse_off_all + (uint64_t)kb * (COARSE + 1);
  const TmpPlanes<WordT> tmp(tmp_all, kb, (uint64_t)MSM_W * bt.cap_m);
  uint32_t* __restrict__ entries = entries_all + (uint64_t)kb * MSM_W * bt.cap_m;
  uint32_t* __restrict__ offsets = offsets_all + (uint64_t)kb * (MSM_NB + 1);
  const uint32_t beg = coff[bin], end = coff[bin + 1];
  if (end - beg > BIG_LIMIT) return;
  if (t < (1u << FINE_BITS)) { cnt[t] = 0; cur[t] = 0; }
  __syncthreads();
  WordT cache[FINE_CACHE > 0 ? FINE_CACHE : 1];
#pragma unroll
  for (uint32_t r = 0; r < FINE_CACHE; ++r) {
    const uint32_t j = beg + t + r * FINE_T;
    cache[r] = j < end ? tmp.ld(j) : (WordT)0;
  }
#pragma unroll
  for (uint32_t r = 0; r < FINE_CACHE; ++r)
    if (beg + t + r * FINE_T < end) atomicAdd(&cnt[SortWord<WordT>::fine(cache[r])], 1u);
  for (uint32_t j = beg + t + FINE_CACHE * FINE_T; j < end; j += FINE_T) atomicAdd(&cnt[tmp.ld_fine(j)], 1u);
  __syncthreads();
  {
    uint32_t total;
    fine_exclusive_scan(cnt, start, scan_tmp, &total);
    if (t < (1u << FINE_BITS)) {
      start[t] += beg;
      offsets[(bin << FINE_BITS) + t] = start[t];
    }
    if (t == 0 && bin == COARSE - 1) offsets[MSM_NB] = beg + total;
    __syncthreads();
  }
  __shared__ uint32_t sorted[(MSM_NB_BITS > 15 && FINE_CACHE > 0) ? FINE_T * FINE_CACHE : 1];
  const bool staged = MSM_NB_BITS > 15 && FINE_CACHE > 0 && end - beg <= FINE_T * FINE_CACHE;
  auto place = [&](WordT e) {
    const uint32_t f = SortWord<WordT>::fine(e);
    const uint32_t pos = start[f] + atomicAdd(&cur[f], 1u);
    if (staged) sorted[pos - beg] = SortWord<WordT>::entry(e);
    else entries[pos] = SortWord<WordT>::entry(e);
  };
#pragma unroll
  for (uint32_t r = 0; r < FINE_CACHE; ++r)
    if (beg + t + r * FINE_T < end) place(cache[r]);
  for (uint32_t j = beg + t + FINE_CACHE * FINE_T; j < end; j += FINE_T) place(tmp.ld(j));
  if (staged) {
    __syncthreads();
    for (uint32_t j = t; j < end - beg; j += FINE_T) entries[beg + j] = sorted[j];
  }
}

__device__ __forceinline__ bool big_item(const uint32_t* __restrict__ big, const uint32_t* __restrict__ coff, uint32_t w,
                                         uint32_t* bin, uint32_t* beg, uint32_t* end) {
  if (w >= big[COARSE]) return false;
  uint32_t lo = 0, hi = COARSE - 1;
  while (lo < hi) {
    const uint32_t mid = (lo + hi + 1) >> 1;
    if (big[mid] <= w) lo = mid; else hi = mid - 1;
  }
  *bin = lo;
  const uint32_t b0 = coff[lo] + (w - big[lo]) * BIG_CHUNK, b1 = coff[lo + 1];
  *beg = b0;
  *end = b0 + BIG_CHUNK < b1 ? b0 + BIG_CHUNK : b1;
  return true;
}
static constexpr uint32_t BIG_T = 512;
static constexpr uint32_t BIG_PER = BIG_CHUNK / BIG_T;
template <class WordT>
__global__ void __launch_bounds__(BIG_T) msm_big_hist_kernel(MsmBatch bt, const uint32_t* __restrict__ coarse_off_all,
                                                             const uint32_t* __restrict__ big_off_all,
                                                             void* __restrict__ tmp_all, uint32_t* __restrict__ big_cnt_all) {
  __shared__ uint32_t cnt[1u << FINE_BITS];
  const int kb = (int)blockIdx.y + bt.kb0;
  const uint32_t* __restrict__ coff = coarse_off_all + (uint64_t)kb * (COARSE + 1);
  const uint32_t* __restrict__ big = big_off_all + (uint64_t)kb * (COARSE + 1);
  const TmpPlanes<WordT> tmp(tmp_all, kb, (uint64_t)MSM_W * bt.cap_m);
  const uint32_t t = threadIdx.x;
  for (uint32_t item = blockIdx.x;; item += gridDim.x) {
    uint32_t bin, beg, end;
    if (!big_item(big, coff, item, &bin, &beg, &end)) return;
    if (t < (1u << FINE_BITS)) cnt[t] = 0;
    __syncthreads();
    for (uint32_t j = beg + t; j < end; j += BIG_T) atomicAdd(&cnt[tmp.ld_fine(j)], 1u);
    __syncthreads();
    if (t < (1u << FINE_BITS) && cnt[t]) atomicAdd(&big_cnt_all[(uint64_t)kb * MSM_NB + (bin << FINE_BITS) + t], cnt[t]);
    __syncthreads();
  }
}
template <class WordT>
__global__ void __launch_bounds__(BIG_T) msm_big_scatter_kernel(MsmBatch bt, const uint32_t* __restrict__ coarse_off_all,
                                                                const uint32_t* __restrict__ big_off_all,
                                                                void* __restrict__ tmp_all,
                                                                const uint32_t* __restrict__ big_cnt_all, uint32_t* __restrict__ big_cur_all,
                                                                uint32_t* __restrict__ entries_all, uint32_t* __restrict__ offsets_all) {
  __shared__ uint32_t cnt[1u << FINE_BITS], base[1u << FINE_BITS], cur[1u << FINE_BITS], bin_cnt[1u << FINE_BITS], scan_tmp[1u << FINE_BITS];
  const int kb = (int)blockIdx.y + bt.kb0;
  const uint32_t* __restrict__ coff = coarse_off_all + (uint64_t)kb * (COARSE + 1);
  const uint32_t* __restrict__ big = big_off_all + (uint64_t)kb * (COARSE + 1);
  const TmpPlanes<WordT> tmp(tmp_all, kb, (uint64_t)MSM_W * bt.cap_m);
  uint32_t* __restrict__ entries = entries_all + (uint64_t)kb * MSM_W * bt.cap_m;
  uint32_t* __restrict__ offsets = offsets_all + (uint64_t)kb * (MSM_NB + 1);
  const uint32_t t = threadIdx.x;
  for (uint32_t item = blockIdx.x;; item += gridDim.x) {
    uint32_t bin, beg, end;
    if (!big_item(big, coff, item, &bin, &beg, &end)) return;
    const uint32_t* __restrict__ bcnt = big_cnt_all + (uint64_t)kb * MSM_NB + (bin << FINE_BITS);
    uint32_t* __restrict__ bcur = big_cur_all + (uint64_t)kb * MSM_NB + (bin << FINE_BITS);
    if (t < (1u << FINE_BITS)) { cnt[t] = 0; cur[t] = 0; }
    __syncthreads();
    WordT cache[BIG_PER];
#pragma unroll
    for (uint32_t r = 0; r < BIG_PER; ++r) {
      const uint32_t j = beg + t + r * BIG_T;
      cache[r] = j < end ? tmp.ld(j) : (WordT)0;
      if (j < end) atomicAdd(&cnt[SortWord<WordT>::fine(cache[r])], 1u);
    }
    __syncthreads();
    {
      const bool first = beg == coff[bin];
      if (t < (1u << FINE_BITS)) bin_cnt[t] = bcnt[t];
      __syncthreads();
      uint32_t total;
      fine_exclusive_scan(bin_cnt, base, scan_tmp, &total);
      if (t < (1u << FINE_BITS)) {
        const uint32_t run = coff[bin] + base[t];
        if (first) offsets[(bin << FINE_BITS) + t] = run;
        base[t] = run + (cnt[t] ? atomicAdd(&bcur[t], cnt[t]) : 0u);
      }
      if (first && t == 0 && bin == COARSE - 1) offsets[MSM_NB] = coff[bin] + total;
    }
    __syncthreads();
#pragma unroll
    for (uint32_t r = 0; r < BIG_PER; ++r) {
      if (beg + t + r * BIG_T < end) {
        const WordT e = cache[r];
        const uint32_t f = SortWord<WordT>::fine(e);
        entries[base[f] + atomicAdd(&cur[f], 1u)] = SortWord<WordT>::entry(e);
      }
    }
    __syncthreads();
  }
}

static constexpr uint32_t HEAVY_SEG_SLICES = 128;
static constexpr uint32_t SLICES_STAGE_WORDS = MSM_NB + MSM_NB / 32 + 2;
static constexpr size_t SLICES_LDS = sizeof(uint32_t) * SLICES_STAGE_WORDS;
__device__ __forceinline__ uint32_t stage_at(uint32_t i) { return i + (i >> 5); }
template <bool ORDER>
__global__ void __launch_bounds__(SORT_T) msm_slices_kernel(const uint32_t* __restrict__ offsets_all,
                                                            uint32_t* __restrict__ slice_off_all, uint32_t ksl, uint32_t heavy_thresh,
                                                            uint32_t* __restrict__ nheavy_all, HeavyItem* __restrict__ heavy_list_all, int kb0,
                                                            uint32_t* __restrict__ full_off_all, uint32_t* __restrict__ part_list_all) {
  extern __shared__ __attribute__((aligned(16))) uint32_t stage[];
  __shared__ uint32_t sh[SORT_T];
  __shared__ uint32_t hist[129];
  const uint32_t* __restrict__ offsets = offsets_all + (uint64_t)(blockIdx.x + (uint32_t)kb0) * (MSM_NB + 1);
  uint32_t* __restrict__ slice_off = slice_off_all + (uint64_t)(blockIdx.x + (uint32_t)kb0) * (MSM_NB + 1);
  uint32_t* __restrict__ nheavy = nheavy_all + 2 * (blockIdx.x + (uint32_t)kb0);
  HeavyItem* __restrict__ heavy_list = heavy_list_all + (uint64_t)(blockIdx.x + (uint32_t)kb0) * MSM_NB;
  constexpr uint32_t PER = MSM_NB / SORT_T;
  const uint32_t t = threadIdx.x;
  for (uint32_t i = t; i <= MSM_NB; i += SORT_T) stage[stage_at(i)] = offsets[i];
  if (ORDER && t < 129) hist[t] = 0;
  __syncthreads();
  uint32_t o[PER + 1];
#pragma unroll
  for (uint32_t k = 0; k <= PER; ++k) o[k] = stage[stage_at(t * PER + k)];
  const uint32_t sh_ksl = 31u - (uint32_t)__builtin_clz(ksl);
  uint32_t mine = 0;
#pragma unroll
  for (uint32_t k = 0; k < PER; ++k) mine += (o[k + 1] - o[k] + ksl - 1) >> sh_ksl;
  uint32_t total;
  uint32_t run = block_exclusive_scan(mine, sh, &total);
#pragma unroll
  for (uint32_t k = 0; k < PER; ++k) {
    stage[stage_at(t * PER + k)] = run;
    const uint32_t ns = (o[k + 1] - o[k] + ksl - 1) >> sh_ksl;
    run += ns;
    if (ns > heavy_thresh) {
      HeavyItem it;
      it.bucket = t * PER + k;
      it.nseg = (ns + HEAVY_SEG_SLICES - 1) / HEAVY_SEG_SLICES;
      it.seg_base = atomicAdd(&nheavy[1], it.nseg);
      it.pad = 0;
      heavy_list[atomicAdd(&nheavy[0], 1u)] = it;
    }
  }
  __syncthreads();
  for (uint32_t i = t; i < MSM_NB; i += SORT_T) slice_off[i] = stage[stage_at(i)];
  if (t == SORT_T - 1) slice_off[MSM_NB] = total;
  if constexpr (ORDER) {
    uint32_t* __restrict__ full_off = full_off_all + (uint64_t)(blockIdx.x + (uint32_t)kb0) * (MSM_NB + 1);
    uint32_t* __restrict__ part_list = part_list_all + (uint64_t)(blockIdx.x + (uint32_t)kb0) * (MSM_NB + 1);
    uint32_t mine_f = 0;
#pragma unroll
    for (uint32_t k = 0; k < PER; ++k) {
      const uint32_t c = o[k + 1] - o[k];
      mine_f += c >> sh_ksl;
      const uint32_t r = c & (ksl - 1);
      if (r) atomicAdd(&hist[r], 1u);
    }
    uint32_t total_f;
    uint32_t run_f = block_exclusive_scan(mine_f, sh, &total_f);
#pragma unroll
    for (uint32_t k = 0; k < PER; ++k) {
      stage[stage_at(t * PER + k)] = run_f;
      run_f += (o[k + 1] - o[k]) >> sh_ksl;
    }
    if (t == 0) {
      uint32_t acc = 0;
      for (uint32_t r = ksl - 1; r >= 1; --r) { const uint32_t h = hist[r]; hist[r] = acc; acc += h; }
      hist[0] = acc;
    }
    __syncthreads();
    for (uint32_t i = t; i < MSM_NB; i += SORT_T) full_off[i] = stage[stage_at(i)];
    if (t == SORT_T - 1) full_off[MSM_NB] = total_f;
#pragma unroll
    for (uint32_t k = 0; k < PER; ++k) {
      const uint32_t r = (o[k + 1] - o[k]) & (ksl - 1);
      if (r) part_list[atomicAdd(&hist[r], 1u)] = t * PER + k;
    }
    if (t == 0) part_list[MSM_NB] = hist[0];
  }
}
#if PLONK_MSM_NB_BITS > 15
static constexpr uint32_t LAY_NBLK = MSM_NB / SORT_T, LAY_H = 132;
static constexpr uint32_t LAY_WORDS = 2 * LAY_NBLK + (LAY_NBLK + 1) * LAY_H;
__global__ void __launch_bounds__(SORT_T) msm_layout_count_kernel(const uint32_t* __restrict__ offsets_all, uint32_t* __restrict__ slice_off_all,
                                                                  uint32_t* __restrict__ full_off_all, uint32_t* __restrict__ lay_all, uint32_t ksl, int kb0) {
  __shared__ uint32_t sh[SORT_T];
  __shared__ uint32_t hist[LAY_H];
  const int kb = (int)blockIdx.y + kb0;
  const uint32_t blk = blockIdx.x, t = threadIdx.x, b = blk * SORT_T + t;
  const uint32_t* __restrict__ offsets = offsets_all + (uint64_t)kb * (MSM_NB + 1);
  uint32_t* __restrict__ lay = lay_all + (uint64_t)kb * LAY_WORDS;
  if (t < LAY_H) hist[t] = 0;
  __syncthreads();
  const uint32_t cnt = offsets[b + 1] - offsets[b];
  const uint32_t nf = cnt / ksl, r = cnt % ksl, ns = nf + (r ? 1u : 0u);
  if (r) atomicAdd(&hist[r], 1u);
  uint32_t tot_ns, tot_nf;
  const uint32_t ex_ns = block_exclusive_scan(ns, sh, &tot_ns);
  const uint32_t ex_nf = block_exclusive_scan(nf, sh, &tot_nf);
  slice_off_all[(uint64_t)kb * (MSM_NB + 1) + b] = ex_ns;
  full_off_all[(uint64_t)kb * (MSM_NB + 1) + b] = ex_nf;
  if (t == 0) { lay[blk] = tot_ns; lay[LAY_NBLK + blk] = tot_nf; }
  if (t < LAY_H) lay[2 * LAY_NBLK + blk * LAY_H + t] = hist[t];
}
__global__ void __launch_bounds__(SORT_T) msm_layout_scan_kernel(uint32_t* __restrict__ slice_off_all, uint32_t* __restrict__ full_off_all,
                                                                 uint32_t* __restrict__ part_list_all, uint32_t* __restrict__ lay_all, uint32_t ksl, int kb0) {
  __shared__ uint32_t sh[SORT_T];
  __shared__ uint32_t ctot[LAY_H];
  const int kb = (blockIdx.x + (uint32_t)kb0);
  const uint32_t t = threadIdx.x;
  uint32_t* __restrict__ lay = lay_all + (uint64_t)kb * LAY_WORDS;
  static_assert(LAY_NBLK <= SORT_T, "one thread per block total");
  uint32_t tot;
  const uint32_t a = t < LAY_NBLK ? lay[t] : 0u;
  const uint32_t ea = block_exclusive_scan(a, sh, &tot);
  if (t < LAY_NBLK) lay[t] = ea;
  if (t == 0) slice_off_all[(uint64_t)kb * (MSM_NB + 1) + MSM_NB] = tot;
  const uint32_t f = t < LAY_NBLK ? lay[LAY_NBLK + t] : 0u;
  const uint32_t ef = block_exclusive_scan(f, sh, &tot);
  if (t < LAY_NBLK) lay[LAY_NBLK + t] = ef;
  if (t == 0) full_off_all[(uint64_t)kb * (MSM_NB + 1) + MSM_NB] = tot;
  if (t < LAY_H) {
    uint32_t run = 0;
    if (t >= 1 && t < ksl)
      for (uint32_t blk = 0; blk < LAY_NBLK; ++blk) {
        uint32_t* q = lay + 2 * LAY_NBLK + blk * LAY_H + t;
        const uint32_t h = *q;
        *q = run;
        run += h;
      }
    ctot[t] = run;
  }
  __syncthreads();
  if (t == 0) {
    uint32_t acc = 0;
    uint32_t* cstart = lay + 2 * LAY_NBLK + LAY_NBLK * LAY_H;
    for (uint32_t r = ksl - 1; r >= 1; --r) { cstart[r] = acc; acc += ctot[r]; }
    part_list_all[(uint64_t)kb * (MSM_NB + 1) + MSM_NB] = acc;
  }
}
__global__ void __launch_bounds__(SORT_T) msm_layout_apply_kernel(const uint32_t* __restrict__ offsets_all, uint32_t* __restrict__ slice_off_all,
                                                                  uint32_t* __restrict__ full_off_all, uint32_t* __restrict__ part_list_all,
                                                                  const uint32_t* __restrict__ lay_all, uint32_t ksl, uint32_t heavy_thresh,
                                                                  uint32_t* __restrict__ nheavy_all, HeavyItem* __restrict__ heavy_list_all,
                                                                  uint4* __restrict__ buckets_raw, uint32_t* __restrict__ multi_list_all, int kb0) {
  __shared__ uint32_t rank[LAY_H];
  const int kb = (int)blockIdx.y + kb0;
  const uint32_t blk = blockIdx.x, t = threadIdx.x, b = blk * SORT_T + t;
  const uint32_t* __restrict__ offsets = offsets_all + (uint64_t)kb * (MSM_NB + 1);
  const uint32_t* __restrict__ lay = lay_all + (uint64_t)kb * LAY_WORDS;
  if (t < LAY_H) rank[t] = 0;
  __syncthreads();
  const uint32_t cnt = offsets[b + 1] - offsets[b];
  const uint32_t nf = cnt / ksl, r = cnt % ksl, ns = nf + (r ? 1u : 0u);
  slice_off_all[(uint64_t)kb * (MSM_NB + 1) + b] += lay[blk];
  full_off_all[(uint64_t)kb * (MSM_NB + 1) + b] += lay[LAY_NBLK + blk];
  if (r) {
    const uint32_t pos = lay[2 * LAY_NBLK + LAY_NBLK * LAY_H + r] + lay[2 * LAY_NBLK + blk * LAY_H + r] + atomicAdd(&rank[r], 1u);
    part_list_all[(uint64_t)kb * (MSM_NB + 1) + pos] = b;
  }
  if (ns > heavy_thresh) {
    HeavyItem it;
    it.bucket = b;
    it.nseg = (ns + HEAVY_SEG_SLICES - 1) / HEAVY_SEG_SLICES;
    it.seg_base = atomicAdd(&nheavy_all[2 * kb + 1], it.nseg);
    it.pad = 0;
    heavy_list_all[(uint64_t)kb * MSM_NB + atomicAdd(&nheavy_all[2 * kb], 1u)] = it;
  } else if (ns == 0) {
    uint4* q = buckets_raw + ((uint64_t)kb * MSM_NB + b) * 16;
#pragma unroll
    for (int k = 0; k < 16; ++k) q[k] = make_uint4(0u, 0u, 0u, 0u);
  }
  __shared__ uint32_t nmul, mbase;
  if (t == 0) nmul = 0;
  __syncthreads();
  const bool multi = ns >= 2 && ns <= heavy_thresh;
  const uint32_t mrank = multi ? atomicAdd(&nmul, 1u) : 0u;
  __syncthreads();
  if (t == 0 && nmul) mbase = atomicAdd(&nheavy_all[2 * MSM_MAX_BATCH + kb], nmul);
  __syncthreads();
  if (multi) multi_list_all[(uint64_t)kb * MSM_NB + mbase + mrank] = b;
}
#endif

int msm_order_slices(Ctx* c, const MsmBatch& bt) {
  (void)c; (void)bt;
  return PLONK_OK;
}

template <int MODE, class WordT>
static int msm_group_sort_t(Ctx* c, const MsmBatch& bt, uint64_t mmax) {
  MsmWork& w = c->msm;
  hipStream_t st = c->stream;
  const uint32_t tiles = (uint32_t)((mmax + TILE - 1) / TILE);
  const uint32_t htiles = (uint32_t)((mmax + HIST_TILE - 1) / HIST_TILE);
  void* tmp = (void*)w.tmp_words;
  const int kb0 = bt.kb0;
  HIP_TRY(hipMemsetAsync(w.coarse_cnt + (size_t)COARSE * kb0, 0, sizeof(uint32_t) * COARSE * bt.count, st));
  hipLaunchKernelGGL(msm_hist_kernel<MODE>, dim3(htiles, bt.count), dim3(SORT_T), 0, st, bt, w.coarse_cnt);
  hipLaunchKernelGGL(msm_coarse_scan_kernel, dim3(bt.count), dim3(SORT_T), 0, st, w.coarse_cnt, w.coarse_off, w.coarse_cur, w.big_off, kb0);
#if PLONK_MSM_NB_BITS >= 19
  if constexpr (MODE != 0) {
    if (c->cfg.sort13 == 1) {
      const uint32_t tiles2 = (uint32_t)((mmax + P2_TILE - 1) / P2_TILE);
      smem_opt_in(c, (const void*)msm_partition2_kernel<MODE, WordT>, PARTITION2_LDS);
      hipLaunchKernelGGL((msm_partition2_kernel<MODE, WordT>), dim3(tiles2, bt.count), dim3(P2_T), PARTITION2_LDS, st, bt, bt.table_n,
                         w.coarse_off, w.coarse_cur, tmp);
    }
  }
  if (MODE == 0 || c->cfg.sort13 != 1) {
#else
  {
#endif
    smem_opt_in(c, (const void*)msm_partition_kernel<MODE, WordT>, PARTITION_LDS);
    hipLaunchKernelGGL((msm_partition_kernel<MODE, WordT>), dim3(tiles, bt.count), dim3(SORT_T), PARTITION_LDS, st, bt, bt.table_n,
                       w.coarse_off, w.coarse_cur, tmp);
  }
  hipLaunchKernelGGL(msm_fine_kernel<WordT>, dim3(COARSE, bt.count), dim3(FINE_T), 0, st, bt, w.coarse_off, tmp,
                     w.entries, w.offsets);
  {
    const uint64_t words = (uint64_t)MSM_W * mmax;
    const uint32_t most = (uint32_t)(words / BIG_CHUNK + words / BIG_LIMIT + 1);
    const uint32_t big_wgs = most < 512u ? most : 512u;
    if (kb0 == 0 && bt.count == bt.group_count) {
      HIP_TRY(hipMemsetAsync(w.big_cnt, 0, sizeof(uint32_t) * 2 * MSM_NB * MSM_MAX_BATCH, st));
    } else {
      HIP_TRY(hipMemsetAsync(w.big_cnt + (size_t)MSM_NB * kb0, 0, sizeof(uint32_t) * MSM_NB * bt.count, st));
      HIP_TRY(hipMemsetAsync(w.big_cnt + (size_t)MSM_NB * MSM_MAX_BATCH + (size_t)MSM_NB * kb0, 0, sizeof(uint32_t) * MSM_NB * bt.count, st));
    }
    hipLaunchKernelGGL(msm_big_hist_kernel<WordT>, dim3(big_wgs, bt.count), dim3(BIG_T), 0, st, bt, w.coarse_off, w.big_off, tmp, w.big_cnt);
    hipLaunchKernelGGL(msm_big_scatter_kernel<WordT>, dim3(big_wgs, bt.count), dim3(BIG_T), 0, st, bt, w.coarse_off, w.big_off, tmp,
                       w.big_cnt, w.big_cnt + (size_t)MSM_NB * MSM_MAX_BATCH, w.entries, w.offsets);
  }
  if (kb0 == 0 && bt.count == bt.group_count) {
    HIP_TRY(hipMemsetAsync(w.nheavy, 0, sizeof(uint32_t) * 4 * MSM_MAX_BATCH, st));
  } else {
    HIP_TRY(hipMemsetAsync(w.nheavy + 2 * kb0, 0, sizeof(uint32_t) * 2 * bt.count, st));
    HIP_TRY(hipMemsetAsync(w.nheavy + 2 * MSM_MAX_BATCH + kb0, 0, sizeof(uint32_t) * bt.count, st));
  }
#if PLONK_MSM_NB_BITS > 15
  if (bt.ksl > 128) return (set_last_error("msm_group_sort", "slice length above 128", __FILE__, __LINE__), PLONK_ERR_ARG);
  hipLaunchKernelGGL(msm_layout_count_kernel, dim3(LAY_NBLK, bt.count), dim3(SORT_T), 0, st, w.offsets, w.slice_off, w.full_off, w.layout, bt.ksl, kb0);
  hipLaunchKernelGGL(msm_layout_scan_kernel, dim3(bt.count), dim3(SORT_T), 0, st, w.slice_off, w.full_off, w.part_list, w.layout, bt.ksl, kb0);
  hipLaunchKernelGGL(msm_layout_apply_kernel, dim3(LAY_NBLK, bt.count), dim3(SORT_T), 0, st, w.offsets, w.slice_off, w.full_off, w.part_list,
                     (const uint32_t*)w.layout, bt.ksl, bt.heavy_thresh, w.nheavy, (HeavyItem*)w.heavy_list, (uint4*)w.buckets, w.multi_list, kb0);
#else
  if (bt.ordered) {
    if (bt.ksl > 128) return (set_last_error("msm_group_sort", "slice length above 128", __FILE__, __LINE__), PLONK_ERR_ARG);
    smem_opt_in(c, (const void*)msm_slices_kernel<true>, SLICES_LDS);
    hipLaunchKernelGGL(msm_slices_kernel<true>, dim3(bt.count), dim3(SORT_T), SLICES_LDS, st, w.offsets, w.slice_off, bt.ksl, bt.heavy_thresh,
                       w.nheavy, (HeavyItem*)w.heavy_list, kb0, w.full_off, w.part_list);
  } else {
    smem_opt_in(c, (const void*)msm_slices_kernel<false>, SLICES_LDS);
    hipLaunchKernelGGL(msm_slices_kernel<false>, dim3(bt.count), dim3(SORT_T), SLICES_LDS, st, w.offsets, w.slice_off, bt.ksl, bt.heavy_thresh,
                       w.nheavy, (HeavyItem*)w.heavy_list, kb0, (uint32_t*)nullptr, (uint32_t*)nullptr);
  }
#endif
  HIP_TRY(hipGetLastError());
  return PLONK_OK;
}
int msm_group_sort(Ctx* c, const MsmBatch& bt, uint64_t mmax) {
  if ((uint64_t)bt.rows * bt.table_n > (1ull << 31))
    return (set_last_error("commit key too large for the bucket sort", "table rows * points must be <= 2^31", __FILE__, __LINE__), PLONK_ERR_ARG);
  if (bt.rows == MSM_ROWS_BITPOS) return bt.wide ? msm_group_sort_t<1, uint64_t>(c, bt, mmax) : msm_group_sort_t<1, uint32_t>(c, bt, mmax);
  if (bt.rows == MSM_ROWS_HALFPOS) return bt.wide ? msm_group_sort_t<2, uint64_t>(c, bt, mmax) : msm_group_sort_t<2, uint32_t>(c, bt, mmax);
#if PLONK_MSM_NB_BITS == 15
  return bt.wide ? msm_group_sort_t<0, uint64_t>(c, bt, mmax) : msm_group_sort_t<0, uint32_t>(c, bt, mmax);
#else
  return (set_last_error("msm_group_sort", "window tables need the 2^15-bucket variant", __FILE__, __LINE__), PLONK_ERR_ARG);
#endif
}
bool msm_needs_wide_words(uint32_t rows, uint64_t table_n) { return (uint64_t)rows * table_n > (1ull << IDX_BITS); }

}
}
```

### plonk_amd/csrc/plonk_internal.hpp

```cpp
#pragma once
#include <hip/hip_runtime.h>
#include <stdint.h>

#include <map>
#include <mutex>
#include <set>
#include <vector>

#include "../../include/plonk_hip.h"
#include "api_guard.hpp"
#include "curve.cuh"
#include "msm_recode.cuh"

#define HIP_TRY(expr)                                                    \
  do {                                                                   \
    hipError_t _e = (expr);                                              \
    if (_e != hipSuccess) {                                              \
      plonk::set_last_error(#expr, hipGetErrorString(_e), __FILE__, __LINE__); \
      return PLONK_ERR_HIP;                                              \
    }                                                                    \
  } while (0)

namespace plonk {

void set_last_error(const char* what, const char* detail, const char* file, int line);
struct Ctx;
int ctx_refuse_poisoned(const char* api_fn);
void finish_pool_release(Ctx* c);
void verify_ws_release(Ctx* c);
bool ctx_abandon(Ctx* c);
#define CTX_ENTER(C, FN)                      \
  std::lock_guard<std::mutex> lk((C).mu);     \
  if ((C).comm_poisoned) return plonk::ctx_refuse_poisoned(FN)

struct NttTables {
  Fr* tw_lo = nullptr;
  Fr* tw_hi = nullptr;
  Fr* tw_lo_scaled = nullptr;
  Fr* w512 = nullptr;
  Fr* g_lo = nullptr;
  Fr* g_hi = nullptr;
  void* tw_lo29 = nullptr;
  void* tw_hi29 = nullptr;
  void* tw_lo_scaled29 = nullptr;
  void* w512_29 = nullptr;
  void* g_lo29 = nullptr;
  void* g_hi29 = nullptr;
  void* tw_a29 = nullptr;
  void* tw_b29 = nullptr;
  Fr n_inv;
};

#ifndef PLONK_MSM_NB_BITS
#define PLONK_MSM_NB_BITS 15
#endif
#if PLONK_MSM_NB_BITS == 15
#define PLONK_MSM_NS nb15
#elif PLONK_MSM_NB_BITS == 17
#define PLONK_MSM_NS nbm
#elif PLONK_MSM_NB_BITS >= 18 && PLONK_MSM_NB_BITS <= 19
#define PLONK_MSM_NS nbl
#else
#error "PLONK_MSM_NB_BITS must be 15 or 17..19"
#endif
static constexpr int MSM_C = 16;
static constexpr int MSM_W = MSM_DIGITS;
static constexpr int MSM_NB_BITS = PLONK_MSM_NB_BITS;
static constexpr uint32_t MSM_NB = 1u << MSM_NB_BITS;
static constexpr int MSM_NB_BITS_MAX = 19;
static constexpr uint32_t MSM_NB_MAX = 1u << MSM_NB_BITS_MAX;
static constexpr uint32_t MSM_NAF_WIDTH = MSM_NB_BITS + 2;
static constexpr int MSM_MAX_BATCH = 4;

struct MsmBatch {
  const Fr* scalars[MSM_MAX_BATCH];
  uint64_t m[MSM_MAX_BATCH];
  G1* out[MSM_MAX_BATCH];
  int count;
  uint32_t ksl;
  uint64_t cap_m, cap_slices;
  const void* table;
  uint64_t table_n;
  uint32_t rows;
  uint32_t ordered;
  uint32_t wide;
  uint32_t heavy_thresh;
  const Fr* tail[MSM_MAX_BATCH];
  uint64_t split[MSM_MAX_BATCH];
  int kb0;
  int group_count;
};

struct HeavyItem { uint32_t bucket, seg_base, nseg, pad; };

struct MsmWork {
  bool fixed_ok = false;
  uint64_t cap_m = 0;
  uint32_t* tmp_words = nullptr;
  uint32_t* entries = nullptr;
  uint32_t* coarse_cnt = nullptr;
  uint32_t* coarse_off = nullptr;
  uint32_t* coarse_cur = nullptr;
  uint32_t* big_off = nullptr;
  uint32_t* big_cnt = nullptr;
  uint32_t* offsets = nullptr;
  uint32_t* slice_off = nullptr;
  uint32_t* full_off = nullptr;
  uint32_t* part_list = nullptr;
  uint32_t* multi_list = nullptr;
  uint32_t* layout = nullptr;
  uint64_t cap_slices = 0;
  void* partial = nullptr;
  void* buckets = nullptr;
  uint32_t* nheavy = nullptr;
  void* heavy_list = nullptr;
  void* seg_sum = nullptr;
  uint64_t cap_segs = 0;
  void* chunk = nullptr;
  int last_rowbits = 8;
  uint8_t* result = nullptr;
  uint8_t* result_host = nullptr;
  Fr* scalars_stage = nullptr;
  uint64_t cap_stage = 0;
};

struct Config {
  uint64_t table_budget = 0;
  int table_mode = 0;
  int bucket_bits = 0;
  int quotient_domain = 4;
  int wire_commit_coeff = 0;
  int z_commit_coeff = 0;
  int shard_quotient = 0;
  int shard_z = 0;
  int shard_side = 0;
  int ntt_elog = 0;
  int comm_timeout_ms = 120000;
  int side_cus = 0;
  int ksl = 0;
  bool prof_fine = false;
  bool acc_lds = false;
  int order = -1;
  bool tail_serial = false;
  bool bsum_lane = false;
  bool rc_lane_tree = false;
  int lps = 0;
  int rcwv = 0;
  int sort13 = -1;
  int acc_wg = 0;
  bool ntt_direct = true;
  int bi_cfg = -1;
  int side_defer = -1;
  int wire_by_column = 0;
  int wire_polys_side = -1;
  int side_after_elog = 0;
  int host_threads = -1;
};

struct plonk_msm_plan_internal {
  uint32_t table_rows = 0, bucket_bits = 0, digit_width = 0, slice_entries = 0, ordered_lanes = 0, wide_words = 0, flags = 0;
  uint64_t terms = 0;
  const char* kernel = "";
};

struct Ctx {
  int device = 0;
  Config cfg;
  uint64_t srs_table_alloc = 0;
  uint64_t table_bytes = 0;
  plonk_msm_plan_internal last_plan;
  hipStream_t stream = nullptr;
  hipStream_t main_stream = nullptr;
  hipStream_t side_stream = nullptr;
  hipEvent_t acc_done = nullptr;
  int ntt_elog_hint = 0;
  std::mutex mu;
  std::mutex table_mu;
  std::map<uint32_t, NttTables*> ntt_tables;
  std::set<const void*> smem_opt_in;
  Fr* ntt_buf = nullptr;
  Fr* ntt_buf2 = nullptr;
  Fr* ntt_buf3 = nullptr;
  hipStream_t copy_stream = nullptr;
  hipStream_t down_stream = nullptr;
  Fr* ntt_tmp = nullptr;
  uint64_t ntt_cap = 0;
  void* srs_table = nullptr;
  uint32_t srs_rows = 0;
  void* table_scratch = nullptr;
  uint64_t table_scratch_pts = 0;
  uint64_t srs_n = 0;
  uint64_t srs_gen = 0;
  MsmWork msm;
  void* nccl_comm = nullptr;
  uint8_t* comm_send = nullptr;
  uint8_t* comm_recv = nullptr;
  uint8_t* comm_send_host = nullptr;
  uint8_t* comm_recv_host = nullptr;
  int comm_rank = 0, comm_world = 1;
  const char* comm_warning = "";
  bool comm_poisoned = false;
  bool comm_loopback = false;
  void* finish_pool = nullptr;
  void* verify_ws = nullptr;
  void* kzg_ws = nullptr;
  bool profile = false;
  hipEvent_t ev0 = nullptr, ev1 = nullptr;
  static constexpr int PROF_SLOTS = 32;
  double acc_ms[PROF_SLOTS] = {0};
  uint64_t acc_n[PROF_SLOTS] = {0};
};

struct NttCoset {
  Fr* g_lo = nullptr;
  Fr* g_hi = nullptr;
  void* g_lo29 = nullptr;
  void* g_hi29 = nullptr;
};
int ntt_coset_tables(Ctx* c, uint32_t L, const Fr& shift, bool inverse, NttCoset* out);
void ntt_coset_free(NttCoset* t);
int ntt_device(Ctx* c, const Fr* src, Fr* dst, Fr* tmp, uint32_t L, bool inverse, bool coset, uint64_t in_len,
               const NttCoset* shift = nullptr);
int ntt_tables(Ctx* c, uint32_t L, bool inverse, NttTables** out);
inline void smem_opt_in(Ctx* c, const void* fn, size_t bytes) {
  if (c->smem_opt_in.insert(fn).second) (void)hipFuncSetAttribute(fn, hipFuncAttributeMaxDynamicSharedMemorySize, (int)bytes);
}
void ntt_plan(uint32_t L, int r[3], int* npass);

struct CommLink {
  int rank = 0, world = 1;
  plonk_allgather_fn fn = nullptr;
  void* user = nullptr;
};
int comm_allgather_host(Ctx* c, const CommLink& l, const void* send, void* recv, size_t bytes);
int comm_sync(Ctx* c, hipStream_t st);
int comm_alltoall_dev(Ctx* c, const CommLink& l, const void* send_dev, void* recv_dev, size_t bytes_per_peer);
int comm_allgather_dev(Ctx* c, const CommLink& l, void* buf_dev, size_t bytes_per_rank);

int srs_load_device(Ctx* c, const G1Affine* pts_dev, uint64_t n);
int srs_table_begin(Ctx* c, uint64_t n);
int srs_table_chunk(Ctx* c, const G1Affine* pts_dev, uint64_t n, uint64_t first, uint64_t count, hipStream_t st);
void srs_table_scratch_free(Ctx* c);
int srs_validate_device(Ctx* c, const G1Affine* pts_dev, uint64_t n, int* flag_dev);
int srs_export_device(Ctx* c, G1Affine* out_dev);
int msm_device(Ctx* c, const Fr* scalars_dev, uint64_t m, G1* out_xyzz_dev);
static constexpr int MSM_BIT_SUMS = 12 + 9;
#define PLONK_MSM_VARIANT_DECLS                                                                                          \
  int msm_order_slices(Ctx* c, const MsmBatch& bt);                                                                      \
  int msm_group_sort(Ctx* c, const MsmBatch& bt, uint64_t mmax);                                                         \
  bool msm_needs_wide_words(uint32_t rows, uint64_t table_n);                                                            \
  int msm_batch_device_v(Ctx* c, MsmBatch& bt, uint64_t mmax, bool bit_sums, int phase);                                 \
  uint32_t msm_ksl(const Ctx* c, uint64_t m);                                                                            \
  bool msm_acc_ordered(const Ctx* c, uint32_t ksl);
namespace nb15 { PLONK_MSM_VARIANT_DECLS }
#ifdef PLONK_MSM_WITH_MEDIUM
namespace nbm { PLONK_MSM_VARIANT_DECLS int msm_buckets_bits(); }
#endif
namespace nbl { PLONK_MSM_VARIANT_DECLS int msm_buckets_bits(); }
int msm_batch_device(Ctx* c, const Fr* const* scalars_dev, const uint64_t* m, int count, G1* const* out_xyzz_dev,
                     bool bit_sums = false, const void* table = nullptr, uint64_t table_n = 0,
                     const Fr* const* tail_dev = nullptr, const uint64_t* split = nullptr, uint32_t table_rows = 0,
                     int phase = 3, int kb0 = 0, int kcount = -1);
uint32_t msm_table_rows(const Ctx* c, uint64_t n, bool last_key);
uint64_t msm_table_bytes(uint32_t rows, uint64_t n);
void msm_plan(const Ctx* c, uint32_t table_rows, uint64_t table_n, uint64_t mmax, int count, bool bit_sums, plonk_msm_plan_internal* out);
void config_resolve(const plonk_gpu_config* user, int device, Config* out);
int srs_table_build(Ctx* c, const G1Affine* pts_dev, uint64_t n, void** table_out, uint32_t* rows_out);
void srs_table_release(Ctx* c, void* table, uint32_t rows, uint64_t n);
int lagrange_points_device(Ctx* c, uint32_t L, G1Affine* out_dev);
int lagrange_blind_points_device(Ctx* c, uint64_t n, uint32_t k0, uint32_t cnt, G1Affine* out_dev);
int xyzz_to_affine97_device(Ctx* c, const G1* in_dev, uint8_t* out97_dev);
void xyzz_to_affine97_host(const G1& p, uint8_t out[97]);
int msm_reserve(Ctx* c, uint64_t m);

struct H1;
struct G1Aff64;
struct G2Prepared;
enum : int { VDEC_OK = 0, VDEC_IDENTITY = 1, VDEC_BAD = 2 };
static constexpr uint32_t VERIFY_MSM_MAX_BLOCKS = 512;
int decode_points(Ctx* c, const uint8_t* comp_host, uint32_t n, uint8_t* comp_dev, G1Affine* pts_dev, int32_t* kind_dev,
                  std::vector<int32_t>* st);
int msm_run(Ctx* c, const uint32_t* sc, const uint32_t* ids, uint64_t nL, uint64_t nR, const G1Affine* pts,
            const int32_t* kind, G1* part_dev, H1 sums[2]);
bool pairing_check(const H1 sums[2], const G2Prepared& x_h, const G2Prepared& h);
G1Aff64 xyzz_to_aff(const H1& p);
int msm_group_sums(Ctx* c, const Fr* const* scalars_dev, const uint64_t* m, int cnt, G1* sums);
void kzg_ws_release(Ctx* c);
int msm_sort_reserve_fixed(Ctx* c);

}

struct plonk_ctx {
  plonk::Ctx c;
};
```

Measured before the change: 30.77.

## Replace MSM histogram pass with pre-provisioned coarse bins and spill handling

```diff
diff --git a/include/plonk_hip.h b/include/plonk_hip.h
--- a/include/plonk_hip.h
+++ b/include/plonk_hip.h
@@ -57,7 +57,7 @@
   uint32_t ordered_lanes;
   uint32_t wide_words;
   uint32_t flags;
-  uint32_t reserved;
+  uint32_t spilled_words;
   uint64_t terms;
   char accumulate_kernel[64];
 } plonk_msm_plan;
diff --git a/plonk_amd/__init__.py b/plonk_amd/__init__.py
--- a/plonk_amd/__init__.py
+++ b/plonk_amd/__init__.py
@@ -87,7 +87,7 @@
 class _MsmPlan(ctypes.Structure):
     _fields_ = [("table_rows", ctypes.c_uint32), ("bucket_bits", ctypes.c_uint32), ("digit_width", ctypes.c_uint32),
                 ("slice_entries", ctypes.c_uint32), ("ordered_lanes", ctypes.c_uint32), ("wide_words", ctypes.c_uint32),
-                ("flags", ctypes.c_uint32), ("reserved", ctypes.c_uint32), ("terms", ctypes.c_uint64), ("accumulate_kernel", ctypes.c_char * 64)]
+                ("flags", ctypes.c_uint32), ("spilled_words", ctypes.c_uint32), ("terms", ctypes.c_uint64), ("accumulate_kernel", ctypes.c_char * 64)]
 
     def as_dict(self) -> dict:
         d = {k: getattr(self, k) for k, _ in self._fields_}
diff --git a/plonk_amd/csrc/capi.hip b/plonk_amd/csrc/capi.hip
--- a/plonk_amd/csrc/capi.hip
+++ b/plonk_amd/csrc/capi.hip
@@ -396,6 +396,12 @@
   std::lock_guard<std::mutex> lk(ctx->c.mu);
   if (!ctx->c.last_plan.table_rows) return (set_last_error("plonk_ctx_last_msm", "no MSM has run on this context", __FILE__, __LINE__), PLONK_ERR_STATE);
   plan_out(ctx->c.last_plan, out);
+  if (ctx->c.msm.spill_ctl && ctx->c.last_plan.group_count > 0) {
+    uint32_t ctl[4 * MSM_MAX_BATCH];
+    for (hipStream_t q : {ctx->c.stream, ctx->c.main_stream, ctx->c.side_stream}) if (q) HIP_TRY(hipStreamSynchronize(q));
+    HIP_TRY(hipMemcpy(ctl, ctx->c.msm.spill_ctl, sizeof(ctl), hipMemcpyDeviceToHost));
+    for (int k = 0; k < ctx->c.last_plan.group_count && k < MSM_MAX_BATCH; ++k) out->spilled_words += ctl[4 * k + 3];
+  }
   return PLONK_OK;
   });
 }
@@ -427,7 +433,7 @@
   if (c.down_stream) (void)hipStreamDestroy(c.down_stream);
   if (c.copy_stream) (void)hipStreamDestroy(c.copy_stream); (void)hipFree(c.srs_table); (void)hipFree(c.table_scratch);
   MsmWork& w = c.msm;
-  (void)hipFree(w.tmp_words); (void)hipFree(w.entries); (void)hipFree(w.coarse_cnt); (void)hipFree(w.coarse_off); (void)hipFree(w.coarse_cur); (void)hipFree(w.big_off); (void)hipFree(w.big_cnt); (void)hipFree(w.nheavy); (void)hipFree(w.heavy_list); (void)hipFree(w.seg_sum);
+  (void)hipFree(w.tmp_words); (void)hipFree(w.entries); (void)hipFree(w.coarse_in); (void)hipFree(w.spill_off); (void)hipFree(w.spill_cur); (void)hipFree(w.spill_ctl); (void)hipFree(w.spill_runs); (void)hipFree(w.coarse_off); (void)hipFree(w.coarse_cur); (void)hipFree(w.big_off); (void)hipFree(w.big_cnt); (void)hipFree(w.nheavy); (void)hipFree(w.heavy_list); (void)hipFree(w.seg_sum);
   (void)hipFree(w.offsets); (void)hipFree(w.slice_off); (void)hipFree(w.full_off); (void)hipFree(w.part_list); (void)hipFree(w.partial); (void)hipFree(w.buckets);
   (void)hipFree(w.multi_list); (void)hipFree(w.layout);
   (void)hipFree(w.chunk); (void)hipFree(w.result); (void)hipFree(w.scalars_stage);
diff --git a/plonk_amd/csrc/msm.hip b/plonk_amd/csrc/msm.hip
--- a/plonk_amd/csrc/msm.hip
+++ b/plonk_amd/csrc/msm.hip
@@ -1311,9 +1311,16 @@
   MsmWork& w = c->msm;
   constexpr int KB = MSM_MAX_BATCH;
   constexpr uint32_t COARSE = 2048;
-  HIP_TRY(hipMalloc((void**)&w.coarse_cnt, sizeof(uint32_t) * COARSE * KB));
+  HIP_TRY(hipMalloc((void**)&w.coarse_in, sizeof(uint32_t) * COARSE * KB));
   HIP_TRY(hipMalloc((void**)&w.coarse_off, sizeof(uint32_t) * (COARSE + 1) * KB));
   HIP_TRY(hipMalloc((void**)&w.coarse_cur, sizeof(uint32_t) * COARSE * KB));
+  HIP_TRY(hipMalloc((void**)&w.spill_off, sizeof(uint32_t) * (COARSE + 1) * KB));
+  HIP_TRY(hipMalloc((void**)&w.spill_cur, sizeof(uint32_t) * COARSE * KB));
+  HIP_TRY(hipMalloc((void**)&w.spill_ctl, sizeof(uint32_t) * 4 * KB));
+  HIP_TRY(hipMemsetAsync(w.coarse_cur, 0, sizeof(uint32_t) * COARSE * KB, c->stream));
+  HIP_TRY(hipMemsetAsync(w.spill_cur, 0, sizeof(uint32_t) * COARSE * KB, c->stream));
+  HIP_TRY(hipMemsetAsync(w.spill_ctl, 0, sizeof(uint32_t) * 4 * KB, c->stream));
+  HIP_TRY(hipStreamSynchronize(c->stream));
   HIP_TRY(hipMalloc((void**)&w.big_off, sizeof(uint32_t) * (COARSE + 1) * KB));
   HIP_TRY(hipMalloc((void**)&w.big_cnt, sizeof(uint32_t) * 2 * MSM_NB_MAX * KB));
   HIP_TRY(hipMalloc((void**)&w.full_off, sizeof(uint32_t) * (MSM_NB_MAX + 1) * KB));
@@ -1327,8 +1334,8 @@
   MsmWork& w = c->msm;
   constexpr int KB = MSM_MAX_BATCH;
   if (!w.fixed_ok) {
-    for (void** q : {(void**)&w.offsets, (void**)&w.slice_off, (void**)&w.nheavy, &w.heavy_list, (void**)&w.coarse_cnt, (void**)&w.coarse_off,
-                     (void**)&w.coarse_cur, (void**)&w.big_off, (void**)&w.big_cnt, (void**)&w.full_off, (void**)&w.part_list, (void**)&w.layout, (void**)&w.multi_list, &w.buckets, &w.chunk,
+    for (void** q : {(void**)&w.offsets, (void**)&w.slice_off, (void**)&w.nheavy, &w.heavy_list, (void**)&w.coarse_in, (void**)&w.coarse_off,
+                     (void**)&w.coarse_cur, (void**)&w.spill_off, (void**)&w.spill_cur, (void**)&w.spill_ctl, (void**)&w.big_off, (void**)&w.big_cnt, (void**)&w.full_off, (void**)&w.part_list, (void**)&w.layout, (void**)&w.multi_list, &w.buckets, &w.chunk,
                      (void**)&w.result}) {
       if (*q) { (void)hipFree(*q); *q = nullptr; }
     }
@@ -1348,10 +1355,11 @@
     const uint64_t cap = m > w.cap_m ? m : w.cap_m;
     HIP_TRY(hipStreamSynchronize(c->stream));
     w.cap_m = 0;
-    for (void** q : {(void**)&w.tmp_words, (void**)&w.entries, (void**)&w.partial, &w.seg_sum}) {
+    for (void** q : {(void**)&w.tmp_words, (void**)&w.entries, (void**)&w.partial, &w.seg_sum, &w.spill_runs}) {
       if (*q) { HIP_TRY(hipFree(*q)); *q = nullptr; }
     }
-    HIP_TRY(hipMalloc((void**)&w.tmp_words, sizeof(uint64_t) * MSM_W * cap * KB));
+    HIP_TRY(hipMalloc((void**)&w.tmp_words, msm_sort_tmp_bytes(cap)));
+    HIP_TRY(hipMalloc(&w.spill_runs, sizeof(uint2) * msm_sort_spill_runs(cap) * KB));
     HIP_TRY(hipMalloc((void**)&w.entries, sizeof(uint32_t) * MSM_W * cap * KB));
     w.cap_slices = msm_slice_cap(c, cap);
     HIP_TRY(hipMalloc((void**)&w.partial, sizeof(G1RSlot) * w.cap_slices * KB));
@@ -1443,6 +1451,7 @@
   }
   plonk_msm_plan_internal plan;
   msm_plan(c, table_rows, table_n, mmax, count, bit_sums, &plan);
+  plan.group_count = count;
   c->last_plan = plan;
   const int nb_bits = (int)plan.bucket_bits;
   if (nb_bits == 19) return nbl::msm_batch_device_v(c, bt, mmax, bit_sums, phase);
diff --git a/plonk_amd/csrc/msm_provision.hpp b/plonk_amd/csrc/msm_provision.hpp
--- /dev/null
+++ b/plonk_amd/csrc/msm_provision.hpp
@@ -0,0 +1,134 @@
+#pragma once
+#include <cmath>
+#include <cstdint>
+#include <mutex>
+
+#include "msm_recode.cuh"
+
+namespace plonk {
+
+static constexpr uint32_t MSM_COARSE_BINS = 2048;
+static constexpr uint32_t MSM_PROV_LEVELS = 24;
+static constexpr uint32_t MSM_PROV_GRAIN = 16;
+static constexpr uint32_t MSM_PROV_R_TOP = 0x73eda753u;
+
+struct MsmProvision {
+  uint32_t cap[MSM_PROV_LEVELS];
+  uint32_t base[MSM_PROV_LEVELS + 1];
+};
+HD uint32_t msm_prov_octave(uint32_t bin) { return bin ? 32u - (uint32_t)__builtin_clz(bin) : 0u; }
+HD uint32_t msm_prov_step_bin(uint32_t octave) { return octave ? MSM_PROV_R_TOP >> (31u - octave) : 0u; }
+HD uint32_t msm_prov_level(uint32_t bin) {
+  const uint32_t l = msm_prov_octave(bin);
+  return 2u * l + (bin > msm_prov_step_bin(l) ? 1u : 0u);
+}
+HD uint32_t msm_prov_level_first(uint32_t level) {
+  const uint32_t l = level >> 1;
+  return (level & 1u) ? msm_prov_step_bin(l) + 1u : (l ? 1u << (l - 1) : 0u);
+}
+HD uint32_t msm_prov_level_bins(uint32_t level) {
+  const uint32_t l = level >> 1, end = l ? 1u << l : 1u;
+  return (level & 1u) ? end - (msm_prov_step_bin(l) + 1u) : (msm_prov_step_bin(l) + 1u) - (l ? 1u << (l - 1) : 0u);
+}
+HD uint32_t msm_prov_cap(const MsmProvision& p, uint32_t bin) { return p.cap[msm_prov_level(bin)]; }
+HD uint32_t msm_prov_base(const MsmProvision& p, uint32_t bin) {
+  const uint32_t v = msm_prov_level(bin);
+  return p.base[v] + (bin - msm_prov_level_first(v)) * p.cap[v];
+}
+
+inline uint32_t msm_prov_digit_width(int mode, int nb_bits) {
+  return mode == 0 ? 16u : (mode == 1 ? (uint32_t)nb_bits + 2u : ((uint32_t)nb_bits + 1u) & ~1u);
+}
+struct MsmProvScalar { uint32_t l[8]; };
+template <class F>
+inline bool msm_prov_recode(int mode, int nb_bits, const MsmProvScalar& s, F&& f) {
+  auto g = [&](int, uint32_t, uint32_t bucket, uint32_t) { f(bucket); };
+  const uint32_t w = msm_prov_digit_width(mode, nb_bits);
+  if (mode == 0 && nb_bits == 15) { for_each_digit_window(s, g); return true; }
+  if (mode == 1) {
+    switch (w) {
+      case 17: for_each_digit_naf<17>(s, g); return true;
+      case 19: for_each_digit_naf<19>(s, g); return true;
+      case 20: for_each_digit_naf<20>(s, g); return true;
+      case 21: for_each_digit_naf<21>(s, g); return true;
+    }
+  }
+  if (mode == 2) {
+    switch (w) {
+      case 16: for_each_digit_even<16>(s, g); return true;
+      case 18: for_each_digit_even<18>(s, g); return true;
+      case 20: for_each_digit_even<20>(s, g); return true;
+    }
+  }
+  return false;
+}
+
+inline const double* msm_prov_density(int mode, int nb_bits) {
+  struct Slot { std::once_flag once; bool ok = false; double d[MSM_PROV_LEVELS]; };
+  static Slot slots[3][5];
+  if (mode < 0 || mode > 2 || nb_bits < 15 || nb_bits > 19) return nullptr;
+  Slot& sl = slots[mode][nb_bits - 15];
+  std::call_once(sl.once, [&] {
+    constexpr uint32_t SAMPLES = 1u << 16;
+    static thread_local uint32_t hist[MSM_COARSE_BINS];
+    for (uint32_t b = 0; b < MSM_COARSE_BINS; ++b) hist[b] = 0;
+    uint64_t x = 0x9e3779b97f4a7c15ull;
+    auto next = [&] {
+      uint64_t z = (x += 0x9e3779b97f4a7c15ull);
+      z = (z ^ (z >> 30)) * 0xbf58476d1ce4e5b9ull;
+      z = (z ^ (z >> 27)) * 0x94d049bb133111ebull;
+      return z ^ (z >> 31);
+    };
+    const uint32_t fine_bits = (uint32_t)nb_bits - 11u;
+    bool ok = true;
+    for (uint32_t i = 0; i < SAMPLES && ok; ++i) {
+      uint64_t q[4];
+      do {
+        for (int k = 0; k < 4; ++k) q[k] = next();
+        q[3] &= 0x7fffffffffffffffull;
+      } while (q[3] >= 0x73eda753299d7d48ull);
+      MsmProvScalar s;
+      for (int k = 0; k < 4; ++k) { s.l[2 * k] = (uint32_t)q[k]; s.l[2 * k + 1] = (uint32_t)(q[k] >> 32); }
+      ok = msm_prov_recode(mode, nb_bits, s, [&](uint32_t bucket) {
+        const uint32_t bin = bucket >> fine_bits;
+        ++hist[bin < MSM_COARSE_BINS ? bin : MSM_COARSE_BINS - 1];
+      });
+    }
+    for (uint32_t v = 0; v < MSM_PROV_LEVELS; ++v) {
+      const uint32_t first = msm_prov_level_first(v), bins = msm_prov_level_bins(v);
+      const uint32_t use = (!(v & 1u) && bins > 1) ? bins - 1 : bins;
+      uint64_t sum = 0;
+      for (uint32_t b = first; b < first + use; ++b) sum += hist[b];
+      sl.d[v] = use ? (double)sum / ((double)SAMPLES * (double)use) : 0.0;
+    }
+    sl.ok = ok;
+  });
+  return sl.ok ? sl.d : nullptr;
+}
+
+inline uint64_t msm_prov_round(double words) { return ((uint64_t)std::ceil(words) + MSM_PROV_GRAIN - 1) / MSM_PROV_GRAIN * MSM_PROV_GRAIN; }
+inline double msm_prov_rule(double mean) { return mean * 1.125 + 8.0 * std::sqrt(mean) + 16.0; }
+
+inline bool msm_provision(int mode, int nb_bits, uint64_t m, MsmProvision* out) {
+  const double* d = msm_prov_density(mode, nb_bits);
+  if (!d) return false;
+  const uint64_t all = msm_prov_round((double)MSM_DIGITS * (double)m);
+  uint64_t base = 0;
+  for (uint32_t l = 0; l < MSM_PROV_LEVELS; ++l) {
+    uint64_t cap = msm_prov_round(msm_prov_rule((double)m * d[l]));
+    if (cap > all) cap = all;
+    out->cap[l] = (uint32_t)cap;
+    out->base[l] = (uint32_t)base;
+    base += cap * msm_prov_level_bins(l);
+    if (base >> 32) return false;
+  }
+  out->base[MSM_PROV_LEVELS] = (uint32_t)base;
+  return true;
+}
+
+inline uint64_t msm_prov_bound(uint64_t m) {
+  const double words = (double)MSM_DIGITS * (double)m;
+  return msm_prov_round(words * 1.125 + 8.0 * std::sqrt((double)MSM_COARSE_BINS * words)) + (uint64_t)MSM_COARSE_BINS * 3 * MSM_PROV_GRAIN   ;
+}
+
+}
diff --git a/plonk_amd/csrc/msm_sort.hip b/plonk_amd/csrc/msm_sort.hip
--- a/plonk_amd/csrc/msm_sort.hip
+++ b/plonk_amd/csrc/msm_sort.hip
@@ -12,12 +12,8 @@
 static constexpr uint32_t TILE = PLONK_SORT_TILE;
 static constexpr uint32_t SORT_T = 1024;
 static constexpr uint32_t PER_T = TILE / SORT_T;
-#ifndef PLONK_HIST_PER
-#define PLONK_HIST_PER 2
-#endif
-static constexpr uint32_t HIST_PER = PLONK_HIST_PER;
-static constexpr uint32_t HIST_TILE = SORT_T * HIST_PER;
 static_assert(COARSE == 2 * SORT_T, "scan / reservation loops assume two coarse bins per thread");
+static_assert(COARSE == MSM_COARSE_BINS, "msm_provision.hpp provisions these bins");
 static constexpr uint32_t IDX_BITS = 31 - FINE_BITS;
 static constexpr uint32_t IDX_MASK = (1u << IDX_BITS) - 1;
 static_assert(IDX_BITS + 1 + FINE_BITS == 32, "narrow intermediate word layout");
@@ -49,6 +45,27 @@
   __device__ __forceinline__ uint32_t ld_fine(uint32_t j) const { return hi[j]; }
   __device__ __forceinline__ void st(uint32_t j, uint64_t w) const { lo[j] = (uint32_t)w; hi[j] = (uint8_t)(w >> 32); }
 };
+template <class WordT> struct RawPlanes;
+template <> struct RawPlanes<uint32_t> {
+  uint32_t* lo;
+  __device__ __forceinline__ RawPlanes(uint32_t* entries_all, void*, int kb, uint64_t words, uint64_t) : lo(entries_all + (uint64_t)kb * words) {}
+  __device__ __forceinline__ uint32_t ld(uint32_t j) const { return lo[j]; }
+  __device__ __forceinline__ void st(uint32_t j, uint32_t w) const { lo[j] = w; }
+};
+template <> struct RawPlanes<uint64_t> {
+  uint32_t* lo;
+  uint8_t* hi;
+  __device__ __forceinline__ RawPlanes(uint32_t* entries_all, void* tmp_all, int kb, uint64_t words, uint64_t stride)
+      : lo(entries_all + (uint64_t)kb * words), hi((uint8_t*)tmp_all + (uint64_t)MSM_MAX_BATCH * stride * 5 + (uint64_t)kb * words) {}
+  __device__ __forceinline__ uint64_t ld(uint32_t j) const { return ((uint64_t)hi[j] << 32) | lo[j]; }
+  __device__ __forceinline__ void st(uint32_t j, uint64_t w) const { lo[j] = (uint32_t)w; hi[j] = (uint8_t)(w >> 32); }
+};
+struct MsmSortPlan {
+  MsmProvision prov[MSM_MAX_BATCH];
+  uint64_t stride;
+};
+static constexpr uint32_t SPILL_CTL = 4;
+static constexpr uint32_t SPILL_FLAG = 0x80000000u;
 static_assert(TILE <= 2048, "tile-local word: 11 bits of scalar index");
 
 __device__ __forceinline__ Fr ld_scalar(const Fr* p);
@@ -71,48 +88,6 @@
 }
 
 static constexpr uint32_t MSM_EVEN_WIDTH = (MSM_NB_BITS + 1) & ~1u;
-template <int MODE>
-__global__ void __launch_bounds__(SORT_T) msm_hist_kernel(MsmBatch bt, uint32_t* __restrict__ coarse_cnt_all) {
-  constexpr bool BITPOS = MODE != 0;
-  __shared__ uint32_t hist[COARSE];
-  __shared__ uint32_t park[BITPOS ? 9 * SORT_T : 1];
-  const int kb = (int)blockIdx.y + bt.kb0;
-  const uint64_t m = bt.m[kb];
-  const uint64_t base = (uint64_t)blockIdx.x * HIST_TILE;
-  if (base >= m) return;
-  const uint32_t t = threadIdx.x;
-  hist[t] = 0;
-  hist[t + SORT_T] = 0;
-  __syncthreads();
-  Fr raw[HIST_PER];
-#pragma unroll
-  for (uint32_t k = 0; k < HIST_PER; ++k) {
-    const uint64_t i = base + t + (uint64_t)k * SORT_T;
-    if (i < m) raw[k] = ld_scalar_at(bt, kb, i);
-  }
-#pragma unroll
-  for (uint32_t k = 0; k < HIST_PER; ++k) {
-    const uint64_t i = base + t + (uint64_t)k * SORT_T;
-    if (i < m) {
-      const Fr s = scalar_canonical(raw[k]);
-      auto count = [&](int, uint32_t, uint32_t bucket, uint32_t) { atomicAdd(&hist[bucket >> FINE_BITS], 1u); };
-      if (BITPOS) {
-#pragma unroll
-        for (int j = 0; j < 8; ++j) park[j * SORT_T + t] = s.l[j];
-        park[8 * SORT_T + t] = 0;
-        if (MODE == 2) for_each_digit_even<MSM_EVEN_WIDTH>(StridedLimbs{park + t, SORT_T}, count);
-        else for_each_digit_naf<MSM_NAF_WIDTH>(StridedLimbs{park + t, SORT_T}, count);
-      } else if constexpr (MSM_NB_BITS == 15) {
-        for_each_digit_window(s, count);
-      }
-    }
-  }
-  __syncthreads();
-  uint32_t* __restrict__ cnt = coarse_cnt_all + (uint64_t)kb * COARSE;
-  const uint32_t a = hist[t], b = hist[t + SORT_T];
-  if (a) atomicAdd(&cnt[t], a);
-  if (b) atomicAdd(&cnt[t + SORT_T], b);
-}
 
 __device__ __forceinline__ uint32_t block_exclusive_scan(uint32_t v, uint32_t* sh , uint32_t* total) {
   const uint32_t t = threadIdx.x;
@@ -151,23 +126,34 @@
 static constexpr uint32_t BIG_CHUNK = 1u << 14;
 __device__ __forceinline__ uint32_t big_chunks(uint32_t cnt) { return cnt > BIG_LIMIT ? (cnt + BIG_CHUNK - 1) / BIG_CHUNK : 0u; }
 
-__global__ void __launch_bounds__(SORT_T) msm_coarse_scan_kernel(const uint32_t* __restrict__ coarse_cnt_all,
-                                                                 uint32_t* __restrict__ coarse_off_all,
-                                                                 uint32_t* __restrict__ coarse_cur_all,
-                                                                 uint32_t* __restrict__ big_off_all, int kb0) {
+__global__ void __launch_bounds__(SORT_T) msm_bins_scan_kernel(MsmSortPlan sp, uint32_t* __restrict__ coarse_cur_all,
+                                                               uint32_t* __restrict__ coarse_in_all,
+                                                               uint32_t* __restrict__ coarse_off_all,
+                                                               uint32_t* __restrict__ big_off_all,
+                                                               uint32_t* __restrict__ spill_off_all,
+                                                               uint32_t* __restrict__ spill_cur_all,
+                                                               uint32_t* __restrict__ spill_ctl_all,
+                                                               uint32_t* __restrict__ nheavy_all, int kb0) {
   __shared__ uint32_t sh[SORT_T];
-  const uint32_t* __restrict__ cnt = coarse_cnt_all + (uint64_t)(blockIdx.x + (uint32_t)kb0) * COARSE;
-  uint32_t* __restrict__ off = coarse_off_all + (uint64_t)(blockIdx.x + (uint32_t)kb0) * (COARSE + 1);
-  uint32_t* __restrict__ cur = coarse_cur_all + (uint64_t)(blockIdx.x + (uint32_t)kb0) * COARSE;
-  uint32_t* __restrict__ big = big_off_all + (uint64_t)(blockIdx.x + (uint32_t)kb0) * (COARSE + 1);
-  const uint32_t t = threadIdx.x;
-  const uint32_t c0 = cnt[2 * t], c1 = cnt[2 * t + 1];
+  const uint32_t kb = blockIdx.x + (uint32_t)kb0;
+  const MsmProvision& pv = sp.prov[kb];
+  uint32_t* __restrict__ cur = coarse_cur_all + (uint64_t)kb * COARSE;
+  uint32_t* __restrict__ in = coarse_in_all + (uint64_t)kb * COARSE;
+  uint32_t* __restrict__ off = coarse_off_all + (uint64_t)kb * (COARSE + 1);
+  uint32_t* __restrict__ big = big_off_all + (uint64_t)kb * (COARSE + 1);
+  uint32_t* __restrict__ soff = spill_off_all + (uint64_t)kb * (COARSE + 1);
+  uint32_t* __restrict__ scur = spill_cur_all + (uint64_t)kb * COARSE;
+  uint32_t* __restrict__ ctl = spill_ctl_all + (uint64_t)kb * SPILL_CTL;
+  const uint32_t t = threadIdx.x;
+  const uint32_t spilled = ctl[0], runs = ctl[1];
+  const uint32_t c0 = cur[2 * t], c1 = cur[2 * t + 1];
+  const uint32_t in0 = c0 <= msm_prov_cap(pv, 2 * t) ? c0 : in[2 * t], in1 = c1 <= msm_prov_cap(pv, 2 * t + 1) ? c1 : in[2 * t + 1];
+  in[2 * t] = in0;
+  in[2 * t + 1] = in1;
   uint32_t total;
   const uint32_t ex = block_exclusive_scan(c0 + c1, sh, &total);
   off[2 * t] = ex;
   off[2 * t + 1] = ex + c0;
-  cur[2 * t] = 0;
-  cur[2 * t + 1] = 0;
   if (t == SORT_T - 1) off[COARSE] = total;
   const uint32_t b0 = big_chunks(c0), b1 = big_chunks(c1);
   uint32_t btotal;
@@ -175,15 +161,44 @@
   big[2 * t] = bex;
   big[2 * t + 1] = bex + b0;
   if (t == SORT_T - 1) big[COARSE] = btotal;
+  if (spilled) {
+    uint32_t stotal;
+    const uint32_t sex = block_exclusive_scan((c0 - in0) + (c1 - in1), sh, &stotal);
+    soff[2 * t] = sex;
+    soff[2 * t + 1] = sex + (c0 - in0);
+    if (t == SORT_T - 1) soff[COARSE] = stotal;
+  }
+  cur[2 * t] = 0;
+  cur[2 * t + 1] = 0;
+  scur[2 * t] = 0;
+  scur[2 * t + 1] = 0;
+  if (t == 0) {
+    ctl[0] = 0; ctl[1] = 0; ctl[2] = runs; ctl[3] = spilled;
+    nheavy_all[2 * kb] = 0; nheavy_all[2 * kb + 1] = 0; nheavy_all[2 * MSM_MAX_BATCH + kb] = 0;
+  }
+}
+
+__device__ __forceinline__ uint32_t reserve_run(const MsmProvision& pv, uint32_t bin, uint32_t c, uint32_t* __restrict__ cur,
+                                                uint32_t* __restrict__ in, uint32_t* __restrict__ ctl, uint2* __restrict__ runs,
+                                                uint32_t* count) {
+  const uint32_t old = atomicAdd(&cur[bin], c), cap = msm_prov_cap(pv, bin);
+  if (old + c <= cap) return msm_prov_base(pv, bin) + old;
+  if (old <= cap) in[bin] = old;
+  const uint32_t at = atomicAdd(&ctl[0], c);
+  runs[atomicAdd(&ctl[1], 1u)] = make_uint2(at, (bin << 16) | c);
+  *count = c | SPILL_FLAG;
+  return at;
 }
 
 static constexpr size_t PARTITION_LDS = ((size_t)TILE * MSM_W + 3 * COARSE) * sizeof(uint32_t);
 
 template <int MODE, class WordT>
-__global__ void __launch_bounds__(SORT_T) msm_partition_kernel(MsmBatch bt, uint64_t srs_n,
-                                                               const uint32_t* __restrict__ coarse_off_all,
+__global__ void __launch_bounds__(SORT_T) msm_partition_kernel(MsmBatch bt, MsmSortPlan sp, uint64_t srs_n,
                                                                uint32_t* __restrict__ coarse_cur_all,
-                                                               void* __restrict__ tmp_all) {
+                                                               uint32_t* __restrict__ coarse_in_all,
+                                                               uint32_t* __restrict__ spill_ctl_all,
+                                                               uint2* __restrict__ spill_runs_all, uint64_t runs_cap,
+                                                               void* __restrict__ tmp_all, uint32_t* __restrict__ entries_all) {
   constexpr bool BITPOS = MODE != 0;
   extern __shared__ __attribute__((aligned(16))) uint32_t lds[];
   uint32_t* stage = lds;
@@ -232,13 +247,16 @@
     const uint32_t ex = block_exclusive_scan(c0 + c1, sh, &total);
     loff[2 * t] = ex;
     loff[2 * t + 1] = ex + c0;
-    const uint32_t* __restrict__ coff = coarse_off_all + (uint64_t)kb * (COARSE + 1);
     uint32_t* __restrict__ cur = coarse_cur_all + (uint64_t)kb * COARSE;
-    gbase[2 * t] = c0 ? coff[2 * t] + atomicAdd(&cur[2 * t], c0) : 0;
-    gbase[2 * t + 1] = c1 ? coff[2 * t + 1] + atomicAdd(&cur[2 * t + 1], c1) : 0;
-  }
-  __syncthreads();
-  const TmpPlanes<WordT> tmp(tmp_all, kb, (uint64_t)MSM_W * bt.cap_m);
+    uint32_t* __restrict__ in = coarse_in_all + (uint64_t)kb * COARSE;
+    uint32_t* __restrict__ ctl = spill_ctl_all + (uint64_t)kb * SPILL_CTL;
+    uint2* __restrict__ runs = spill_runs_all + (uint64_t)kb * runs_cap;
+    gbase[2 * t] = c0 ? reserve_run(sp.prov[kb], 2 * t, c0, cur, in, ctl, runs, &hist[2 * t]) : 0;
+    gbase[2 * t + 1] = c1 ? reserve_run(sp.prov[kb], 2 * t + 1, c1, cur, in, ctl, runs, &hist[2 * t + 1]) : 0;
+  }
+  __syncthreads();
+  const TmpPlanes<WordT> tmp(tmp_all, kb, sp.stride);
+  const RawPlanes<WordT> raw(entries_all, tmp_all, kb, (uint64_t)MSM_W * bt.cap_m, sp.stride);
 #pragma unroll
   for (uint32_t k = 0; k < PER_T; ++k)
 #pragma unroll
@@ -247,10 +265,11 @@
   __syncthreads();
   const uint32_t sub = t & 15;
   for (uint32_t bin = t >> 4; bin < COARSE; bin += SORT_T / 16) {
-    const uint32_t cnt = hist[bin], lo = loff[bin], gb = gbase[bin];
+    const uint32_t h = hist[bin], cnt = h & ~SPILL_FLAG, lo = loff[bin], gb = gbase[bin];
     for (uint32_t j = sub; j < cnt; j += 16) {
       const uint32_t lw = stage[lo + j];
-      tmp.st(gb + j, SortWord<WordT>::make(lw >> 20, (lw >> 19) & 1u, (uint64_t)((lw >> 11) & 0xffu) * srs_n + base + (lw & 0x7ffu)));
+      const WordT gw = SortWord<WordT>::make(lw >> 20, (lw >> 19) & 1u, (uint64_t)((lw >> 11) & 0xffu) * srs_n + base + (lw & 0x7ffu));
+      if (h & SPILL_FLAG) raw.st(gb + j, gw); else tmp.st(gb + j, gw);
     }
   }
 }
@@ -278,10 +297,12 @@
 }
 
 template <int MODE, class WordT>
-__global__ void __launch_bounds__(P2_T, 4) msm_partition2_kernel(MsmBatch bt, uint64_t srs_n,
-                                                                  const uint32_t* __restrict__ coarse_off_all,
+__global__ void __launch_bounds__(P2_T, 4) msm_partition2_kernel(MsmBatch bt, MsmSortPlan sp, uint64_t srs_n,
                                                                   uint32_t* __restrict__ coarse_cur_all,
-                                                                  void* __restrict__ tmp_all) {
+                                                                  uint32_t* __restrict__ coarse_in_all,
+                                                                  uint32_t* __restrict__ spill_ctl_all,
+                                                                  uint2* __restrict__ spill_runs_all, uint64_t runs_cap,
+                                                                  void* __restrict__ tmp_all, uint32_t* __restrict__ entries_all) {
   static_assert(MODE != 0, "bit-position / half-density recodings only");
   extern __shared__ __attribute__((aligned(16))) uint32_t lds[];
   uint32_t* stage = lds;
@@ -328,18 +349,21 @@
     for (uint32_t j = 0; j < P2_BPT; ++j) { cnt[j] = hist[P2_BPT * t + j]; sum += cnt[j]; }
     uint32_t total;
     uint32_t run = block_exclusive_scan_p2(sum, sh, &total);
-    const uint32_t* __restrict__ coff = coarse_off_all + (uint64_t)kb * (COARSE + 1);
     uint32_t* __restrict__ cur = coarse_cur_all + (uint64_t)kb * COARSE;
+    uint32_t* __restrict__ in = coarse_in_all + (uint64_t)kb * COARSE;
+    uint32_t* __restrict__ ctl = spill_ctl_all + (uint64_t)kb * SPILL_CTL;
+    uint2* __restrict__ runs = spill_runs_all + (uint64_t)kb * runs_cap;
 #pragma unroll
     for (uint32_t j = 0; j < P2_BPT; ++j) {
       const uint32_t bin = P2_BPT * t + j;
       loff[bin] = run;
       run += cnt[j];
-      gbase[bin] = cnt[j] ? coff[bin] + atomicAdd(&cur[bin], cnt[j]) : 0;
-    }
-  }
-  __syncthreads();
-  const TmpPlanes<WordT> tmp(tmp_all, kb, (uint64_t)MSM_W * bt.cap_m);
+      gbase[bin] = cnt[j] ? reserve_run(sp.prov[kb], bin, cnt[j], cur, in, ctl, runs, &hist[bin]) : 0;
+    }
+  }
+  __syncthreads();
+  const TmpPlanes<WordT> tmp(tmp_all, kb, sp.stride);
+  const RawPlanes<WordT> raw(entries_all, tmp_all, kb, (uint64_t)MSM_W * bt.cap_m, sp.stride);
 #pragma unroll
   for (uint32_t k = 0; k < P2_PER; ++k)
 #pragma unroll
@@ -348,14 +372,56 @@
   __syncthreads();
   const uint32_t sub = t & 7;
   for (uint32_t bin = t >> 3; bin < COARSE; bin += P2_T / 8) {
-    const uint32_t cnt = hist[bin], lo = loff[bin], gb = gbase[bin];
+    const uint32_t h = hist[bin], cnt = h & ~SPILL_FLAG, lo = loff[bin], gb = gbase[bin];
     for (uint32_t j = sub; j < cnt; j += 8) {
       const uint32_t lw = stage[lo + j];
-      tmp.st(gb + j, SortWord<WordT>::make(lw >> 20, (lw >> 19) & 1u, (uint64_t)((lw >> 11) & 0xffu) * srs_n + base + (lw & 0x7ffu)));
+      const WordT gw = SortWord<WordT>::make(lw >> 20, (lw >> 19) & 1u, (uint64_t)((lw >> 11) & 0xffu) * srs_n + base + (lw & 0x7ffu));
+      if (h & SPILL_FLAG) raw.st(gb + j, gw); else tmp.st(gb + j, gw);
     }
   }
 }
 #endif
+
+static constexpr uint32_t SPILL_T = 256, SPILL_WG = 256;
+template <class WordT>
+__global__ void __launch_bounds__(SPILL_T) msm_spill_scatter_kernel(MsmBatch bt, MsmSortPlan sp, const uint32_t* __restrict__ spill_off_all,
+                                                                    uint32_t* __restrict__ spill_cur_all,
+                                                                    const uint32_t* __restrict__ spill_ctl_all,
+                                                                    const uint2* __restrict__ spill_runs_all, uint64_t runs_cap,
+                                                                    void* __restrict__ tmp_all, uint32_t* __restrict__ entries_all) {
+  const int kb = (int)blockIdx.y + bt.kb0;
+  const uint32_t nruns = spill_ctl_all[(uint64_t)kb * SPILL_CTL + 2];
+  if (!nruns) return;
+  const uint32_t* __restrict__ soff = spill_off_all + (uint64_t)kb * (COARSE + 1);
+  uint32_t* __restrict__ scur = spill_cur_all + (uint64_t)kb * COARSE;
+  const uint2* __restrict__ runs = spill_runs_all + (uint64_t)kb * runs_cap;
+  const TmpPlanes<WordT> tmp(tmp_all, kb, sp.stride);
+  const RawPlanes<WordT> raw(entries_all, tmp_all, kb, (uint64_t)MSM_W * bt.cap_m, sp.stride);
+  const uint32_t behind = sp.prov[kb].base[MSM_PROV_LEVELS];
+  const uint32_t lane = threadIdx.x & 63u, wave = threadIdx.x >> 6;
+  for (uint32_t r = blockIdx.x * (SPILL_T / 64) + wave; r < nruns; r += gridDim.x * (SPILL_T / 64)) {
+    const uint2 d = runs[r];
+    const uint32_t bin = d.y >> 16, cnt = d.y & 0xffffu;
+    uint32_t at = 0;
+    if (lane == 0) at = atomicAdd(&scur[bin], cnt);
+    at = (uint32_t)__shfl((int)at, 0);
+    const uint32_t dst = behind + soff[bin] + at;
+    for (uint32_t j = lane; j < cnt; j += 64) tmp.st(dst + j, raw.ld(d.x + j));
+  }
+}
+
+struct BinMap {
+  uint32_t in, pb, sb;
+  __device__ __forceinline__ uint32_t operator()(uint32_t i) const { return i < in ? pb + i : sb + (i - in); }
+};
+__device__ __forceinline__ BinMap bin_map(const MsmSortPlan& sp, int kb, uint32_t bin, const uint32_t* __restrict__ coarse_in_all,
+                                          const uint32_t* __restrict__ spill_off_all) {
+  BinMap mp;
+  mp.in = coarse_in_all[(uint64_t)kb * COARSE + bin];
+  mp.pb = msm_prov_base(sp.prov[kb], bin);
+  mp.sb = sp.prov[kb].base[MSM_PROV_LEVELS] + spill_off_all[(uint64_t)kb * (COARSE + 1) + bin];
+  return mp;
+}
 
 #ifndef PLONK_FINE_T
 #define PLONK_FINE_T 512
@@ -366,7 +432,9 @@
 static constexpr uint32_t FINE_T = PLONK_FINE_T;
 static constexpr uint32_t FINE_CACHE = PLONK_FINE_CACHE;
 template <class WordT>
-__global__ void __launch_bounds__(FINE_T) msm_fine_kernel(MsmBatch bt, const uint32_t* __restrict__ coarse_off_all,
+__global__ void __launch_bounds__(FINE_T) msm_fine_kernel(MsmBatch bt, MsmSortPlan sp, const uint32_t* __restrict__ coarse_off_all,
+                                                          const uint32_t* __restrict__ coarse_in_all,
+                                                          const uint32_t* __restrict__ spill_off_all,
                                                           void* __restrict__ tmp_all,
                                                           uint32_t* __restrict__ entries_all,
                                                           uint32_t* __restrict__ offsets_all) {
@@ -374,23 +442,24 @@
   const int kb = (int)blockIdx.y + bt.kb0;
   const uint32_t bin = blockIdx.x, t = threadIdx.x;
   const uint32_t* __restrict__ coff = coarse_off_all + (uint64_t)kb * (COARSE + 1);
-  const TmpPlanes<WordT> tmp(tmp_all, kb, (uint64_t)MSM_W * bt.cap_m);
+  const TmpPlanes<WordT> tmp(tmp_all, kb, sp.stride);
   uint32_t* __restrict__ entries = entries_all + (uint64_t)kb * MSM_W * bt.cap_m;
   uint32_t* __restrict__ offsets = offsets_all + (uint64_t)kb * (MSM_NB + 1);
-  const uint32_t beg = coff[bin], end = coff[bin + 1];
-  if (end - beg > BIG_LIMIT) return;
+  const uint32_t beg = coff[bin], n = coff[bin + 1] - beg;
+  if (n > BIG_LIMIT) return;
+  const BinMap at = bin_map(sp, kb, bin, coarse_in_all, spill_off_all);
   if (t < (1u << FINE_BITS)) { cnt[t] = 0; cur[t] = 0; }
   __syncthreads();
   WordT cache[FINE_CACHE > 0 ? FINE_CACHE : 1];
 #pragma unroll
   for (uint32_t r = 0; r < FINE_CACHE; ++r) {
-    const uint32_t j = beg + t + r * FINE_T;
-    cache[r] = j < end ? tmp.ld(j) : (WordT)0;
+    const uint32_t i = t + r * FINE_T;
+    cache[r] = i < n ? tmp.ld(at(i)) : (WordT)0;
   }
 #pragma unroll
   for (uint32_t r = 0; r < FINE_CACHE; ++r)
-    if (beg + t + r * FINE_T < end) atomicAdd(&cnt[SortWord<WordT>::fine(cache[r])], 1u);
-  for (uint32_t j = beg + t + FINE_CACHE * FINE_T; j < end; j += FINE_T) atomicAdd(&cnt[tmp.ld_fine(j)], 1u);
+    if (t + r * FINE_T < n) atomicAdd(&cnt[SortWord<WordT>::fine(cache[r])], 1u);
+  for (uint32_t i = t + FINE_CACHE * FINE_T; i < n; i += FINE_T) atomicAdd(&cnt[tmp.ld_fine(at(i))], 1u);
   __syncthreads();
   {
     uint32_t total;
@@ -403,7 +472,7 @@
     __syncthreads();
   }
   __shared__ uint32_t sorted[(MSM_NB_BITS > 15 && FINE_CACHE > 0) ? FINE_T * FINE_CACHE : 1];
-  const bool staged = MSM_NB_BITS > 15 && FINE_CACHE > 0 && end - beg <= FINE_T * FINE_CACHE;
+  const bool staged = MSM_NB_BITS > 15 && FINE_CACHE > 0 && n <= FINE_T * FINE_CACHE;
   auto place = [&](WordT e) {
     const uint32_t f = SortWord<WordT>::fine(e);
     const uint32_t pos = start[f] + atomicAdd(&cur[f], 1u);
@@ -412,11 +481,11 @@
   };
 #pragma unroll
   for (uint32_t r = 0; r < FINE_CACHE; ++r)
-    if (beg + t + r * FINE_T < end) place(cache[r]);
-  for (uint32_t j = beg + t + FINE_CACHE * FINE_T; j < end; j += FINE_T) place(tmp.ld(j));
+    if (t + r * FINE_T < n) place(cache[r]);
+  for (uint32_t i = t + FINE_CACHE * FINE_T; i < n; i += FINE_T) place(tmp.ld(at(i)));
   if (staged) {
     __syncthreads();
-    for (uint32_t j = t; j < end - beg; j += FINE_T) entries[beg + j] = sorted[j];
+    for (uint32_t j = t; j < n; j += FINE_T) entries[beg + j] = sorted[j];
   }
 }
 
@@ -437,28 +506,34 @@
 static constexpr uint32_t BIG_T = 512;
 static constexpr uint32_t BIG_PER = BIG_CHUNK / BIG_T;
 template <class WordT>
-__global__ void __launch_bounds__(BIG_T) msm_big_hist_kernel(MsmBatch bt, const uint32_t* __restrict__ coarse_off_all,
+__global__ void __launch_bounds__(BIG_T) msm_big_hist_kernel(MsmBatch bt, MsmSortPlan sp, const uint32_t* __restrict__ coarse_off_all,
+                                                             const uint32_t* __restrict__ coarse_in_all,
+                                                             const uint32_t* __restrict__ spill_off_all,
                                                              const uint32_t* __restrict__ big_off_all,
                                                              void* __restrict__ tmp_all, uint32_t* __restrict__ big_cnt_all) {
   __shared__ uint32_t cnt[1u << FINE_BITS];
   const int kb = (int)blockIdx.y + bt.kb0;
   const uint32_t* __restrict__ coff = coarse_off_all + (uint64_t)kb * (COARSE + 1);
   const uint32_t* __restrict__ big = big_off_all + (uint64_t)kb * (COARSE + 1);
-  const TmpPlanes<WordT> tmp(tmp_all, kb, (uint64_t)MSM_W * bt.cap_m);
+  const TmpPlanes<WordT> tmp(tmp_all, kb, sp.stride);
   const uint32_t t = threadIdx.x;
   for (uint32_t item = blockIdx.x;; item += gridDim.x) {
     uint32_t bin, beg, end;
     if (!big_item(big, coff, item, &bin, &beg, &end)) return;
     if (t < (1u << FINE_BITS)) cnt[t] = 0;
     __syncthreads();
-    for (uint32_t j = beg + t; j < end; j += BIG_T) atomicAdd(&cnt[tmp.ld_fine(j)], 1u);
+    const BinMap at = bin_map(sp, kb, bin, coarse_in_all, spill_off_all);
+    const uint32_t first = coff[bin];
+    for (uint32_t j = beg + t; j < end; j += BIG_T) atomicAdd(&cnt[tmp.ld_fine(at(j - first))], 1u);
     __syncthreads();
     if (t < (1u << FINE_BITS) && cnt[t]) atomicAdd(&big_cnt_all[(uint64_t)kb * MSM_NB + (bin << FINE_BITS) + t], cnt[t]);
     __syncthreads();
   }
 }
 template <class WordT>
-__global__ void __launch_bounds__(BIG_T) msm_big_scatter_kernel(MsmBatch bt, const uint32_t* __restrict__ coarse_off_all,
+__global__ void __launch_bounds__(BIG_T) msm_big_scatter_kernel(MsmBatch bt, MsmSortPlan sp, const uint32_t* __restrict__ coarse_off_all,
+                                                                const uint32_t* __restrict__ coarse_in_all,
+                                                                const uint32_t* __restrict__ spill_off_all,
                                                                 const uint32_t* __restrict__ big_off_all,
                                                                 void* __restrict__ tmp_all,
                                                                 const uint32_t* __restrict__ big_cnt_all, uint32_t* __restrict__ big_cur_all,
@@ -467,7 +542,7 @@
   const int kb = (int)blockIdx.y + bt.kb0;
   const uint32_t* __restrict__ coff = coarse_off_all + (uint64_t)kb * (COARSE + 1);
   const uint32_t* __restrict__ big = big_off_all + (uint64_t)kb * (COARSE + 1);
-  const TmpPlanes<WordT> tmp(tmp_all, kb, (uint64_t)MSM_W * bt.cap_m);
+  const TmpPlanes<WordT> tmp(tmp_all, kb, sp.stride);
   uint32_t* __restrict__ entries = entries_all + (uint64_t)kb * MSM_W * bt.cap_m;
   uint32_t* __restrict__ offsets = offsets_all + (uint64_t)kb * (MSM_NB + 1);
   const uint32_t t = threadIdx.x;
@@ -478,11 +553,12 @@
     uint32_t* __restrict__ bcur = big_cur_all + (uint64_t)kb * MSM_NB + (bin << FINE_BITS);
     if (t < (1u << FINE_BITS)) { cnt[t] = 0; cur[t] = 0; }
     __syncthreads();
+    const BinMap at = bin_map(sp, kb, bin, coarse_in_all, spill_off_all);
     WordT cache[BIG_PER];
 #pragma unroll
     for (uint32_t r = 0; r < BIG_PER; ++r) {
       const uint32_t j = beg + t + r * BIG_T;
-      cache[r] = j < end ? tmp.ld(j) : (WordT)0;
+      cache[r] = j < end ? tmp.ld(at(j - coff[bin])) : (WordT)0;
       if (j < end) atomicAdd(&cnt[SortWord<WordT>::fine(cache[r])], 1u);
     }
     __syncthreads();
@@ -707,19 +783,23 @@
   MsmWork& w = c->msm;
   hipStream_t st = c->stream;
   const uint32_t tiles = (uint32_t)((mmax + TILE - 1) / TILE);
-  const uint32_t htiles = (uint32_t)((mmax + HIST_TILE - 1) / HIST_TILE);
   void* tmp = (void*)w.tmp_words;
   const int kb0 = bt.kb0;
-  HIP_TRY(hipMemsetAsync(w.coarse_cnt + (size_t)COARSE * kb0, 0, sizeof(uint32_t) * COARSE * bt.count, st));
-  hipLaunchKernelGGL(msm_hist_kernel<MODE>, dim3(htiles, bt.count), dim3(SORT_T), 0, st, bt, w.coarse_cnt);
-  hipLaunchKernelGGL(msm_coarse_scan_kernel, dim3(bt.count), dim3(SORT_T), 0, st, w.coarse_cnt, w.coarse_off, w.coarse_cur, w.big_off, kb0);
+  MsmSortPlan sp{};
+  sp.stride = msm_sort_tmp_stride(bt.cap_m);
+  if (sp.stride >> 32) return (set_last_error("msm_group_sort", "too many terms for 32-bit word positions", __FILE__, __LINE__), PLONK_ERR_ARG);
+  for (int k = kb0; k < kb0 + bt.count; ++k)
+    if (!msm_provision(MODE, MSM_NB_BITS, bt.m[k], &sp.prov[k]) || sp.prov[k].base[MSM_PROV_LEVELS] > msm_prov_bound(bt.cap_m))
+      return (set_last_error("msm_group_sort", "provisioned bins exceed the word buffer", __FILE__, __LINE__), PLONK_ERR_ARG);
+  const uint64_t runs_cap = msm_sort_spill_runs(bt.cap_m);
+  uint2* runs = (uint2*)w.spill_runs;
 #if PLONK_MSM_NB_BITS >= 19
   if constexpr (MODE != 0) {
     if (c->cfg.sort13 == 1) {
       const uint32_t tiles2 = (uint32_t)((mmax + P2_TILE - 1) / P2_TILE);
       smem_opt_in(c, (const void*)msm_partition2_kernel<MODE, WordT>, PARTITION2_LDS);
-      hipLaunchKernelGGL((msm_partition2_kernel<MODE, WordT>), dim3(tiles2, bt.count), dim3(P2_T), PARTITION2_LDS, st, bt, bt.table_n,
-                         w.coarse_off, w.coarse_cur, tmp);
+      hipLaunchKernelGGL((msm_partition2_kernel<MODE, WordT>), dim3(tiles2, bt.count), dim3(P2_T), PARTITION2_LDS, st, bt, sp, bt.table_n,
+                         w.coarse_cur, w.coarse_in, w.spill_ctl, runs, runs_cap, tmp, w.entries);
     }
   }
   if (MODE == 0 || c->cfg.sort13 != 1) {
@@ -727,10 +807,14 @@
   {
 #endif
     smem_opt_in(c, (const void*)msm_partition_kernel<MODE, WordT>, PARTITION_LDS);
-    hipLaunchKernelGGL((msm_partition_kernel<MODE, WordT>), dim3(tiles, bt.count), dim3(SORT_T), PARTITION_LDS, st, bt, bt.table_n,
-                       w.coarse_off, w.coarse_cur, tmp);
-  }
-  hipLaunchKernelGGL(msm_fine_kernel<WordT>, dim3(COARSE, bt.count), dim3(FINE_T), 0, st, bt, w.coarse_off, tmp,
+    hipLaunchKernelGGL((msm_partition_kernel<MODE, WordT>), dim3(tiles, bt.count), dim3(SORT_T), PARTITION_LDS, st, bt, sp, bt.table_n,
+                       w.coarse_cur, w.coarse_in, w.spill_ctl, runs, runs_cap, tmp, w.entries);
+  }
+  hipLaunchKernelGGL(msm_bins_scan_kernel, dim3(bt.count), dim3(SORT_T), 0, st, sp, w.coarse_cur, w.coarse_in, w.coarse_off, w.big_off,
+                     w.spill_off, w.spill_cur, w.spill_ctl, w.nheavy, kb0);
+  hipLaunchKernelGGL(msm_spill_scatter_kernel<WordT>, dim3(tiles < SPILL_WG ? tiles : SPILL_WG, bt.count), dim3(SPILL_T), 0, st, bt, sp,
+                     w.spill_off, w.spill_cur, w.spill_ctl, (const uint2*)runs, runs_cap, tmp, w.entries);
+  hipLaunchKernelGGL(msm_fine_kernel<WordT>, dim3(COARSE, bt.count), dim3(FINE_T), 0, st, bt, sp, w.coarse_off, w.coarse_in, w.spill_off, tmp,
                      w.entries, w.offsets);
   {
     const uint64_t words = (uint64_t)MSM_W * mmax;
@@ -742,15 +826,9 @@
       HIP_TRY(hipMemsetAsync(w.big_cnt + (size_t)MSM_NB * kb0, 0, sizeof(uint32_t) * MSM_NB * bt.count, st));
       HIP_TRY(hipMemsetAsync(w.big_cnt + (size_t)MSM_NB * MSM_MAX_BATCH + (size_t)MSM_NB * kb0, 0, sizeof(uint32_t) * MSM_NB * bt.count, st));
     }
-    hipLaunchKernelGGL(msm_big_hist_kernel<WordT>, dim3(big_wgs, bt.count), dim3(BIG_T), 0, st, bt, w.coarse_off, w.big_off, tmp, w.big_cnt);
-    hipLaunchKernelGGL(msm_big_scatter_kernel<WordT>, dim3(big_wgs, bt.count), dim3(BIG_T), 0, st, bt, w.coarse_off, w.big_off, tmp,
+    hipLaunchKernelGGL(msm_big_hist_kernel<WordT>, dim3(big_wgs, bt.count), dim3(BIG_T), 0, st, bt, sp, w.coarse_off, w.coarse_in, w.spill_off, w.big_off, tmp, w.big_cnt);
+    hipLaunchKernelGGL(msm_big_scatter_kernel<WordT>, dim3(big_wgs, bt.count), dim3(BIG_T), 0, st, bt, sp, w.coarse_off, w.coarse_in, w.spill_off, w.big_off, tmp,
                        w.big_cnt, w.big_cnt + (size_t)MSM_NB * MSM_MAX_BATCH, w.entries, w.offsets);
-  }
-  if (kb0 == 0 && bt.count == bt.group_count) {
-    HIP_TRY(hipMemsetAsync(w.nheavy, 0, sizeof(uint32_t) * 4 * MSM_MAX_BATCH, st));
-  } else {
-    HIP_TRY(hipMemsetAsync(w.nheavy + 2 * kb0, 0, sizeof(uint32_t) * 2 * bt.count, st));
-    HIP_TRY(hipMemsetAsync(w.nheavy + 2 * MSM_MAX_BATCH + kb0, 0, sizeof(uint32_t) * bt.count, st));
   }
 #if PLONK_MSM_NB_BITS > 15
   if (bt.ksl > 128) return (set_last_error("msm_group_sort", "slice length above 128", __FILE__, __LINE__), PLONK_ERR_ARG);
diff --git a/plonk_amd/csrc/plonk_internal.hpp b/plonk_amd/csrc/plonk_internal.hpp
--- a/plonk_amd/csrc/plonk_internal.hpp
+++ b/plonk_amd/csrc/plonk_internal.hpp
@@ -11,6 +11,7 @@
 #include "api_guard.hpp"
 #include "curve.cuh"
 #include "msm_recode.cuh"
+#include "msm_provision.hpp"
 
 #define HIP_TRY(expr)                                                    \
   do {                                                                   \
@@ -91,6 +92,10 @@
   int group_count;
 };
 
+inline uint64_t msm_sort_tmp_stride(uint64_t cap_m) { return msm_prov_bound(cap_m) + (uint64_t)MSM_W * cap_m; }
+inline uint64_t msm_sort_tmp_bytes(uint64_t cap_m) { return (uint64_t)MSM_MAX_BATCH * (5 * msm_sort_tmp_stride(cap_m) + (uint64_t)MSM_W * cap_m); }
+inline uint64_t msm_sort_spill_runs(uint64_t cap_m) { return (uint64_t)MSM_COARSE_BINS * ((cap_m + 1023) / 1024); }
+
 struct HeavyItem { uint32_t bucket, seg_base, nseg, pad; };
 
 struct MsmWork {
@@ -98,9 +103,13 @@
   uint64_t cap_m = 0;
   uint32_t* tmp_words = nullptr;
   uint32_t* entries = nullptr;
-  uint32_t* coarse_cnt = nullptr;
+  uint32_t* coarse_in = nullptr;
   uint32_t* coarse_off = nullptr;
   uint32_t* coarse_cur = nullptr;
+  uint32_t* spill_off = nullptr;
+  uint32_t* spill_cur = nullptr;
+  uint32_t* spill_ctl = nullptr;
+  void* spill_runs = nullptr;
   uint32_t* big_off = nullptr;
   uint32_t* big_cnt = nullptr;
   uint32_t* offsets = nullptr;
@@ -159,6 +168,7 @@
 
 struct plonk_msm_plan_internal {
   uint32_t table_rows = 0, bucket_bits = 0, digit_width = 0, slice_entries = 0, ordered_lanes = 0, wide_words = 0, flags = 0;
+  int group_count = 0;
   uint64_t terms = 0;
   const char* kernel = "";
 };
```

Result: no change. 30.79 (median of 2 runs) (+0.1%).
